# oceanbase/oceanbase

Hardware: AMD Instinct MI355X
Metric: rows/sec, TPC-H lineitem scan->filter->agg (microblock decode + pushdown filter + group-by) (higher is better)
Workload: dtype int64; 1 GPU; tpch_q1_sf100_lineitem_scan_filter_agg; rows_per_gpu=600000000, total_rows=600000000, encoded_bytes_per_gpu=7341603792, n_blocks=453858, block_bytes=16384

## Files before the change

include/obx.h:

```cpp
#ifndef OBX_H_
#define OBX_H_

#include <stdint.h>
#include <stddef.h>

#ifdef __cplusplus
extern "C" {
#endif

enum {
  OBX_SUCCESS = 0,
  OBX_ITER_END = -4008,
  OBX_INVALID_ARGUMENT = -4002,
  OBX_NOT_SUPPORTED = -4007,
  OBX_BUF_NOT_ENOUGH = -4009,
  OBX_NO_GPU = -7001,
  OBX_INTERNAL_ERROR = -4016,
  OBX_PHYSIC_CHECKSUM_ERROR = -4108,
};

enum obx_encoding {
  OBX_ENC_RAW = 0,
  OBX_ENC_DICT = 1,
  OBX_ENC_RLE = 2,
// ... 59 lines not shown
  const obx_col_schema *cols;
  uint64_t total_rows;
} obx_blockset;

#define OBX_MAX_IN_LIST 8
typedef struct obx_filter_leaf {
  uint16_t col;
  uint8_t op;
  uint8_t n_in;
  int64_t lo;
  int64_t hi;
  int64_t in_list[OBX_MAX_IN_LIST];
  int64_t bconst[OBX_BX_MAX_CONST];
  uint16_t bcols[OBX_BX_MAX_COLS];
  uint8_t n_bprog;
  uint8_t n_bcols;
  uint8_t bprog[OBX_BX_MAX_PROG];
  uint8_t bpad[6];
} obx_filter_leaf;

#define OBX_TOK_AND 128
#define OBX_TOK_OR 129
#define OBX_MAX_PROG 15

typedef struct obx_filter_desc {
  uint16_t n_leaves;
  uint8_t n_prog;
  uint8_t prog[OBX_MAX_PROG];
  obx_filter_leaf leaves[8];
} obx_filter_desc;

typedef struct obx_agg_expr {
  uint8_t kind;
  uint16_t col_a;
  uint16_t col_b;
  uint16_t col_c;
} obx_agg_expr;

typedef struct obx_agg_desc {
  uint8_t n_group_cols;
  uint16_t group_cols[2];
  uint8_t n_aggs;
  obx_agg_expr aggs[8];
} obx_agg_desc;

typedef struct obx_agg_cell { uint64_t limb[4]; } obx_agg_cell;

#define OBX_MAX_GROUPS 64
#define OBX_MAX_KEY_BYTES 16
typedef struct obx_group_row {
  uint8_t key[OBX_MAX_KEY_BYTES];
  uint8_t key_len;
  uint64_t row_count;
  obx_agg_cell cells[8];
} obx_group_row;

typedef struct obx_agg_result {
  uint32_t n_groups;
  obx_group_row groups[OBX_MAX_GROUPS];
  uint64_t rows_scanned;
  uint64_t rows_passed;
} obx_agg_result;

typedef struct obx_batch {
  uint64_t *skip_bits;
  int64_t size;
  uint8_t end;
  uint8_t all_rows_active;
} obx_batch;


int64_t obx_encode_block(const obx_col_schema *cols, uint16_t n_cols,
                         const uint8_t *const *col_data,
                         const uint8_t *const *null_bitmaps,
                         uint32_t row_count, const uint8_t *enc_request,
                         uint8_t *out, int64_t out_cap);

uint64_t obx_crc32c(const uint8_t *buf, int64_t len);

int obx_decode_block(const obx_col_schema *cols, uint16_t n_cols,
                     const uint8_t *block, int64_t block_len,
                     const uint16_t *proj_cols, uint16_t n_proj,
                     uint8_t *const *out_cols, uint8_t *const *out_nulls,
                     uint32_t *row_count);

int obx_cpu_filter_block(const obx_col_schema *cols, uint16_t n_cols,
                         const uint8_t *block, int64_t block_len,
                         const obx_filter_desc *filter,
                         uint8_t *result_bits, uint32_t *row_count,
                         uint32_t *popcnt);

int obx_cpu_scan_filter_agg(const obx_blockset *bs,
                            const obx_filter_desc *filter,
                            const obx_agg_desc *agg,
                            int nthreads,
                            obx_agg_result *out);

int64_t obx_gen_lineitem(int config, uint64_t row_count, uint64_t seed,
                         uint32_t target_block_bytes,
                         uint64_t row_id_base,
                         uint8_t **out_data, uint64_t **out_offsets,
                         obx_col_schema *out_cols, uint16_t *out_n_cols);

typedef struct obx_gpu_ctx obx_gpu_ctx;

int obx_gpu_open(int device, obx_gpu_ctx **ctx);
int obx_gpu_close(obx_gpu_ctx *ctx);

int obx_gpu_load_blocks(obx_gpu_ctx *ctx, const obx_blockset *bs);

int obx_gpu_load_cs_blocks(obx_gpu_ctx *ctx, const obx_blockset *bs);

int obx_cs_host_parse(const uint8_t *buf, int64_t len, uint32_t *rows_out,
                      uint32_t *ncols_out);
int obx_gpu_free_blocks(obx_gpu_ctx *ctx, int handle);

int obx_gpu_filter(obx_gpu_ctx *ctx, int handle, const obx_filter_desc *filter,
                   int want_row_ids);
int obx_gpu_fetch_bitmap(obx_gpu_ctx *ctx, int handle, uint8_t *out, int64_t cap);
int obx_gpu_fetch_row_ids(obx_gpu_ctx *ctx, int handle, int32_t *out,
                          int64_t cap, uint64_t *n_out);
int obx_gpu_fetch_blk_counts(obx_gpu_ctx *ctx, int handle, uint32_t *out,
                             int64_t cap);

int obx_gpu_decode(obx_gpu_ctx *ctx, int handle, const uint16_t *proj_cols,
                   uint16_t n_proj);
int obx_gpu_fetch_col(obx_gpu_ctx *ctx, int handle, uint16_t col,
                      uint8_t *out, int64_t cap);

int obx_gpu_scan_project(obx_gpu_ctx *ctx, int handle,
                         const obx_filter_desc *filter,
                         const uint16_t *proj_cols, uint16_t n_proj,
                         int want_row_nos, uint64_t *n_rows);

int obx_gpu_fetch_proj(obx_gpu_ctx *ctx, int handle, uint16_t proj_idx,
                       uint64_t start, uint64_t count,
                       uint8_t *out, int64_t cap,
                       uint8_t *out_nulls, int64_t nulls_cap, uint64_t *n_out);

int obx_gpu_fetch_proj_row_nos(obx_gpu_ctx *ctx, int handle, uint64_t start,
                               uint64_t count, uint64_t *out, int64_t cap,
                               uint64_t *n_out);

double obx_gpu_last_proj_stage_ms(obx_gpu_ctx *ctx, int stage);

int obx_gpu_scan_filter_agg(obx_gpu_ctx *ctx, int handle,
                            const obx_filter_desc *filter,
                            const obx_agg_desc *agg,
                            obx_agg_result *out);

double obx_gpu_last_kernel_ms(obx_gpu_ctx *ctx);
double obx_gpu_last_prep_ms(obx_gpu_ctx *ctx);
int obx_gpu_last_jit(obx_gpu_ctx *ctx);
uint32_t obx_gpu_last_grid(obx_gpu_ctx *ctx);
uint64_t obx_gpu_total_rows(obx_gpu_ctx *ctx, int handle);
uint64_t obx_gpu_total_bytes(obx_gpu_ctx *ctx, int handle);
uint64_t obx_gpu_last_survivors(obx_gpu_ctx *ctx, int handle);

int obx_gpu_agg_fetch(obx_gpu_ctx *ctx, int handle, uint32_t start,
                      uint32_t count, obx_group_row *out, uint32_t *n_out,
                      uint64_t *n_total);
int obx_cpu_agg_fetch(uint32_t start, uint32_t count, obx_group_row *out,
                      uint32_t *n_out, uint64_t *n_total);

int64_t obx_jit_dump_src(const obx_filter_desc *filter,
                         const obx_agg_desc *agg,
                         const obx_col_schema *cols, uint16_t n_cols,
                         const uint8_t *col_flags, const int64_t *col_min,
                         const int64_t *col_max, const uint32_t *col_maxcnt,
                         const uint32_t *col_maxw, uint32_t max_block_rows,
                         int force_v1, char *out, int64_t cap);

#ifdef __cplusplus
}
#endif
#endif
```

oceanbase_amd/csrc/obx_dev.h:

```cpp
#ifndef OBX_DEV_H_
#define OBX_DEV_H_

#if defined(__HIPRTC__) || defined(OBX_HIPRTC)
typedef signed char int8_t;
typedef unsigned char uint8_t;
typedef short int16_t;
typedef unsigned short uint16_t;
typedef int int32_t;
typedef unsigned int uint32_t;
typedef long long int64_t;
typedef unsigned long long uint64_t;
typedef unsigned long size_t;
#define INT64_MAX 0x7fffffffffffffffll
#define INT64_MIN (-INT64_MAX - 1ll)
#define UINT64_MAX 0xffffffffffffffffull
#else
#include <stdint.h>
#endif

#define OBX_DEV_MAX_COLS 8
#define OBX_DEV_MAX_LEAVES 8
#define OBX_DEV_MAX_AGGS 8
#define OBX_GTABLE_SLOTS 256
#define OBX_GTABLE_SHIFT 8
#define OBX_GTABLE_BIG 4096
#define OBX_GTABLE_BIG_SHIFT 12
#define OBX_LTABLE_SLOTS 16

enum {
  OBX_D_RAW = 0,
  OBX_D_DICT = 1,
  OBX_D_RLE = 2,
  OBX_D_CONST = 3,
  OBX_D_INTDIFF = 4,
  OBX_D_SDIFF = 5,
  OBX_D_HEX = 6,
  OBX_D_SPREFIX = 7,
  OBX_D_EQUAL = 8,
  OBX_D_SUBSTR = 9,
};

enum {
  OBX_DF_BITPACK = 1,
  OBX_DF_HAS_EXT = 2,
  OBX_DF_SIGNED = 4,
  OBX_DF_STRING = 8,
};

typedef struct dev_col {
  uint64_t data_bit;
  uint64_t ext_bit;
  uint64_t dict_byte;
  uint64_t aux_byte;
  int64_t base;
  uint32_t count;
  uint32_t runs;
  uint8_t enc;
  uint8_t flags;
  uint8_t width;
  uint8_t entry_len;
  uint8_t rib, rfb;
  uint8_t datum_len;
  uint8_t ext_width;
  uint8_t tss;
  uint8_t pad[7];
} dev_col;

typedef struct dev_block {
  uint32_t row_start_lo;
  uint32_t row_start_hi;
  uint32_t row_count;
  uint32_t block_len;
  uint64_t block_byte;
  dev_col cols[OBX_DEV_MAX_COLS];
} dev_block;

#define OBX_LDS_STAGE_BYTES 17408

#if defined(__HIPCC__) || defined(__HIP_DEVICE_COMPILE__)
__host__ __device__
#endif
static inline uint64_t dev_block_row_start(const dev_block *b) {
  return ((uint64_t)b->row_start_hi << 32) | b->row_start_lo;
}

enum {
  OBX_LEAF_NONE = 0,
  OBX_LEAF_ALL = 1,
  OBX_LEAF_REF_MASK = 2,
  OBX_LEAF_RANGE = 3,
  OBX_LEAF_VALUE = 4,
  OBX_LEAF_NULL = 5,
};

typedef struct dev_leaf {
  int64_t vlo, vhi;
  uint16_t col;
  uint8_t op;
  uint8_t n_in;
  uint8_t char_len;
  uint8_t pad[3];
  int64_t in_list[8];
  int64_t bconst[4];
  uint16_t bcols[4];
  uint8_t n_bprog;
  uint8_t n_bcols;
  uint8_t bprog[24];
  uint8_t bpad[6];
} dev_leaf;

typedef struct blk_leaf {
  uint64_t mask;
  uint64_t lo, hi;
  uint8_t mode;
  uint8_t invert;
  uint8_t pad[6];
} blk_leaf;

typedef struct dev_agg {
  uint8_t kind;
  uint8_t ia, ib, ic;
  int32_t pad;
  int64_t one_b, one_c;
} dev_agg;

#define OBX_DEV_MAX_NEED 12

typedef struct dev_pass_agg {
  uint8_t kind;
  uint8_t agg_idx;
  uint8_t sa, sb, sc;
  uint8_t pad[3];
  int64_t one_b, one_c;
} dev_pass_agg;

typedef struct dev_pass {
  uint8_t n_aggs;
  uint8_t n_cols;
  uint8_t cols[3];
  uint8_t pad[3];
  dev_pass_agg aggs[OBX_DEV_MAX_AGGS];
} dev_pass;

typedef struct dev_plan_hdr {
  uint32_t n_leaves;
  uint32_t n_aggs;
  uint32_t n_group_cols;
  uint32_t n_need;
  uint32_t n_passes;
  uint8_t n_prog;
  uint8_t prog[15];
  uint16_t need_cols[OBX_DEV_MAX_NEED];
  uint8_t group_idx[2];
  uint8_t group_len[2];
  dev_agg aggs[OBX_DEV_MAX_AGGS];
  dev_pass passes[OBX_DEV_MAX_AGGS];
} dev_plan_hdr;

typedef struct gslot {
  unsigned long long key;
  unsigned long long count;
  unsigned long long cells[OBX_DEV_MAX_AGGS][4];
} gslot;

#define OBX_KEY_EMPTY 0xFFFFFFFFFFFFFFFFull

#endif
```

oceanbase_amd/csrc/obx_engine.cpp:

```cpp
#include <cstdlib>
#include <cstring>
#include <algorithm>

#include "obx_host.h"

#define OBX_RESULT_BYTES(slots) (sizeof(gslot) * (slots) + 16 * 8)

extern "C" int obx_gpu_open(int device, obx_gpu_ctx **out) {
  int n = 0;
  hipError_t e = hipGetDeviceCount(&n);
  if (e != hipSuccess || n <= device) return OBX_NO_GPU;
  auto *ctx = new obx_gpu_ctx();
  ctx->device = device;
  HIP_TRY(hipSetDevice(device));
  HIP_TRY(hipStreamCreate(&ctx->stream));
  HIP_TRY(hipEventCreate(&ctx->ev_start));
  HIP_TRY(hipEventCreate(&ctx->ev_stop));
  HIP_TRY(hipEventCreate(&ctx->ev_p0));
  HIP_TRY(hipEventCreate(&ctx->ev_p1));
  HIP_TRY(hipEventCreate(&ctx->ev_mid));
  {
    hipDeviceProp_t prop;
    HIP_TRY(hipGetDeviceProperties(&prop, device));
    if (prop.multiProcessorCount > 0)
      ctx->n_cus = (uint32_t)prop.multiProcessorCount;
  }
  HIP_TRY(hipHostMalloc((void **)&ctx->h_result,
                        OBX_RESULT_BYTES(OBX_GTABLE_BIG), hipHostMallocDefault));
  *out = ctx;
  return OBX_SUCCESS;
}

extern "C" int obx_gpu_close(obx_gpu_ctx *ctx) {
  if (!ctx) return OBX_SUCCESS;
  (void)hipSetDevice(ctx->device);
  ctx->handles.clear();
  (void)hipStreamDestroy(ctx->stream);
  for (hipEvent_t ev : {ctx->ev_start, ctx->ev_stop, ctx->ev_p0, ctx->ev_p1,
                        ctx->ev_mid})
    (void)hipEventDestroy(ev);
  (void)hipHostFree(ctx->h_result);
  delete ctx;
  return OBX_SUCCESS;
}

obx_handle::~obx_handle() {
  void *owned[] = {d_buf, d_blocks, d_bleaves, d_pleaves, d_gtable,
                   d_gtable_big, d_proj_scratch, d_bitmap, d_row_ids,
                   d_blk_counts, d_row_slot, d_minmax, d_sel_nulls,
                   d_sel_row_nos, d_blk_off, d_tile_sums, d_sel_bits};
  for (void *p : owned)
    if (p) (void)hipFree(p);
  for (uint8_t *p : d_decode_out)
    if (p) (void)hipFree(p);
  for (uint8_t *p : d_sel_out)
    if (p) (void)hipFree(p);
}

static obx_handle *lookup(obx_gpu_ctx *ctx, int handle) {
  if (!ctx || handle < 0 || handle >= (int)ctx->handles.size()) return nullptr;
  return ctx->handles[handle].get();
}

__attribute__((target("sse4.2")))
static uint64_t host_crc32c(const uint8_t *buf, int64_t len) {
  uint64_t crc = 0;
  int64_t i = 0;
  for (; i + 8 <= len; i += 8) {
    uint64_t w;
    memcpy(&w, buf + i, 8);
    crc = __builtin_ia32_crc32di(crc, w);
  }
  for (; i < len; i++) crc = __builtin_ia32_crc32qi((uint32_t)crc, buf[i]);
  return crc;
}

#define OBX_JIT_GRID_WAVES 8
static uint32_t jit_grid_for(uint32_t n_blocks, uint32_t n_cus, int wpb) {
  uint64_t g = (uint64_t)(n_cus ? n_cus : 1) * (uint32_t)(wpb > 0 ? wpb : 1) *
               OBX_JIT_GRID_WAVES;
  if (g > n_blocks) g = n_blocks;
  return g ? (uint32_t)g : 1;
}

static void gtable_init(gslot *gt, uint32_t n_slots, uint32_t tail_words,
                        uint32_t min_mask, uint32_t max_mask,
                        hipStream_t stream) {
  const uint32_t words =
      n_slots * (uint32_t)(sizeof(gslot) / 8) + tail_words;
  hipLaunchKernelGGL(k_gtable_init, dim3((words + OBX_WG_HOST - 1) / OBX_WG_HOST),
                     dim3(OBX_WG_HOST), 0, stream, (unsigned long long *)gt,
                     n_slots, tail_words, min_mask, max_mask);
}

static void summarize_col_classes(obx_handle &h) {
  const uint32_t nc = h.n_cols;
  const bool first = h.col_class.size() == nc;
  const uint8_t *cls = h.col_class.data() + h.col_class.size() - nc;
  const uint8_t *cnt = h.col_cnt.data() + h.col_cnt.size() - nc;
  for (uint32_t c = 0; c < nc; c++) {
    const uint8_t k = cls[c];
    if (first) h.col_grp16_every[c] = true;
    if ((k & 0xF) == 5) h.col_span_any[c] = true;
    if ((k & 0xF) != 1 || cnt[c] >= 16) h.col_grp16_every[c] = false;
    if ((k & 0xF) > 3 || (k & 0x10)) h.col_slow_any[c] = true;
    if (cnt[c] > h.col_cnt_max[c]) h.col_cnt_max[c] = cnt[c];
  }
}

void obx_fold_block(obx_handle &h, const dev_block &db) {
  const bool first = h.col_class.empty();
  if ((db.block_byte & 15) ||
      (uint64_t)db.block_len + 24 > OBX_LDS_STAGE_BYTES ||
      db.row_count > 4096 )
    h.lds_ok = false;
  for (uint16_t c = 0; c < h.n_cols; c++) {
    const dev_col &dc = db.cols[c];
    uint8_t cls;
    switch (dc.enc) {
      case OBX_D_RAW: cls = 0; break;
      case OBX_D_DICT: cls = 1; break;
      case OBX_D_INTDIFF: cls = 2; break;
      case OBX_D_CONST: cls = dc.runs == 0 ? 3 : 4; break;
      case OBX_D_EQUAL: case OBX_D_SUBSTR:
        cls = 5; break;
      default: cls = 4; break;
    }
    if (dc.flags & OBX_DF_STRING) cls |= 0x10;
    h.col_class.push_back(cls);
    h.col_cnt.push_back((uint8_t)(dc.count > 254 ? 255 : dc.count));
    if (first) {
      h.col_dict_every[c] = true;
      h.col_dict_any[c] = true;
      h.col_raw8_every[c] = true;
      h.col_rangefam_every[c] = true;
    }
    if ((cls & 0xF) != 1 || (cls & 0x10) || dc.count > 63)
      h.col_dict_every[c] = false;
    if ((cls & 0xF) != 1 || dc.count > 63)
      h.col_dict_any[c] = false;
    if (!(dc.enc == OBX_D_RAW && !(dc.flags & OBX_DF_BITPACK) &&
          !(dc.flags & OBX_DF_STRING) && !(dc.flags & OBX_DF_HAS_EXT) &&
          dc.width == 8 && (dc.data_bit & 63) == 0))
      h.col_raw8_every[c] = false;
    if (!((dc.enc == OBX_D_RAW || dc.enc == OBX_D_INTDIFF) &&
          !(dc.flags & OBX_DF_STRING) && !(dc.flags & OBX_DF_HAS_EXT)))
      h.col_rangefam_every[c] = false;
    if (dc.count > h.col_maxcnt[c]) h.col_maxcnt[c] = dc.count;
    if (dc.flags & OBX_DF_HAS_EXT) h.col_ext_any[c] = true;
    uint32_t w = 255;
    if (dc.enc == OBX_D_RAW || dc.enc == OBX_D_DICT || dc.enc == OBX_D_INTDIFF)
      w = (dc.flags & OBX_DF_BITPACK) ? dc.width : (uint32_t)dc.width * 8;
    if (w > h.col_maxw[c]) h.col_maxw[c] = w;
  }
  summarize_col_classes(h);
  if (db.row_count > h.max_block_rows) h.max_block_rows = db.row_count;
  if (db.block_len > h.max_block_len) h.max_block_len = db.block_len;
  h.n_blocks++;
  h.total_rows += db.row_count;
}

static int parse_block(const obx_col_schema *cols, uint16_t n_cols,
                       const uint8_t *block, uint64_t dev_off,
                       uint64_t block_len, uint64_t row_start,
                       dev_block *out) {
  const obx_micro_header *h = (const obx_micro_header *)block;
  if (h->magic != OBX_MICRO_BLOCK_MAGIC) return OBX_INVALID_ARGUMENT;
  if (h->column_count != n_cols) return OBX_INVALID_ARGUMENT;
  if (h->data_zlength > (int64_t)block_len ||
      h->data_zlength < OBX_MICRO_HEADER_SIZE)
    return OBX_INVALID_ARGUMENT;
  if ((int64_t)host_crc32c(block + OBX_MICRO_HEADER_SIZE,
                           (int64_t)h->data_zlength - OBX_MICRO_HEADER_SIZE) !=
      h->data_checksum)
    return OBX_PHYSIC_CHECKSUM_ERROR;
  memset(out, 0, sizeof(*out));
  out->row_start_lo = (uint32_t)row_start;
  out->row_start_hi = (uint32_t)(row_start >> 32);
  out->row_count = h->row_count;
  out->block_len = (uint32_t)block_len;
  out->block_byte = dev_off;
  const uint64_t meta_base =
      dev_off + h->header_size + (uint64_t)n_cols * sizeof(obx_col_header);
  const obx_col_header *chp =
      (const obx_col_header *)(block + h->header_size);
  const uint8_t *meta_host = block + h->header_size +
                             (uint64_t)n_cols * sizeof(obx_col_header);
  const uint8_t evb = obx_hdr_extend_value_bit(h);

  for (uint16_t c = 0; c < n_cols; c++) {
    const obx_col_header *ch = &chp[c];
    dev_col *dc = &out->cols[c];
    const int sc = obx_store_class(ch->obj_type);
    const int64_t tss = obx_type_store_size(ch->obj_type);
    dc->enc = (uint8_t)ch->type;
    dc->datum_len = cols[c].len;
    dc->tss = (uint8_t)(tss > 0 ? tss : cols[c].len);
    dc->ext_width = evb;
    if (sc == OBX_SC_INT) dc->flags |= OBX_DF_SIGNED;
    if (sc == OBX_SC_STRING) dc->flags |= OBX_DF_STRING;
    const uint64_t col_base = meta_base + ch->offset;
    const uint8_t *col_host = meta_host + ch->offset;
    const int has_ext = (ch->attr & OBX_COL_ATTR_HAS_EXTEND_VALUE) ? 1 : 0;
    const int bp = (ch->attr & OBX_COL_ATTR_BIT_PACKING) ? 1 : 0;

    switch (ch->type) {
      case OBX_COL_RAW: {
        if (bp) dc->flags |= OBX_DF_BITPACK;
        dc->width = (uint8_t)ch->length;
        uint64_t ext_bits = has_ext ? (uint64_t)evb * h->row_count : 0;
        if (has_ext) {
          dc->flags |= OBX_DF_HAS_EXT;
          dc->ext_bit = col_base * 8;
        }
        if (bp) {
          dc->data_bit = col_base * 8 + ext_bits;
        } else {
          dc->data_bit = (col_base + (ext_bits + 7) / 8) * 8;
        }
        break;
      }
      case OBX_COL_DICT: {
        const obx_dict_meta *dm = (const obx_dict_meta *)col_host;
        if (bp) dc->flags |= OBX_DF_BITPACK;
        dc->width = dm->row_ref_size;
        dc->count = dm->count;
        dc->entry_len = (uint8_t)dm->data_size;
        dc->dict_byte = col_base + sizeof(obx_dict_meta);
        dc->data_bit = (col_base + ch->length) * 8;
        break;
      }
      case OBX_COL_RLE: {
        const obx_rle_meta *rm = (const obx_rle_meta *)col_host;
        dc->runs = rm->count;
        dc->rib = rm->attr & 7;
        dc->rfb = (rm->attr >> 3) & 7;
        dc->aux_byte = col_base + sizeof(obx_rle_meta);
        const obx_dict_meta *dm =
            (const obx_dict_meta *)(col_host + rm->offset);
        dc->count = dm->count;
        dc->entry_len = (uint8_t)dm->data_size;
        dc->dict_byte = col_base + rm->offset + sizeof(obx_dict_meta);
        break;
      }
      case OBX_COL_CONST: {
        const obx_const_meta *cm = (const obx_const_meta *)col_host;
        dc->runs = cm->count;
        dc->rib = cm->attr & 7;
        dc->rfb = cm->const_ref;
        if (cm->count == 0) {
          if (cm->const_ref > 0) {
            dc->count = 0;
          } else {
            dc->count = 1;
            int64_t cell = (sc == OBX_SC_INT) ? tss : cols[c].len;
            uint64_t v = 0;
            memcpy(&v, col_host + cm->offset, (size_t)cell);
            dc->base = (sc == OBX_SC_INT)
                           ? (int64_t)obx_sign_extend(v, tss, 1)
                           : (sc == OBX_SC_DECIMAL
                                  ? (int64_t)obx_sign_extend(v, cell, 1)
                                  : (int64_t)v);
          }
        } else {
          dc->aux_byte = col_base + sizeof(obx_const_meta);
          const obx_dict_meta *dm =
              (const obx_dict_meta *)(col_host + cm->offset);
          dc->count = dm->count;
          dc->entry_len = (uint8_t)dm->data_size;
          dc->dict_byte = col_base + cm->offset + sizeof(obx_dict_meta);
        }
        break;
      }
      case OBX_COL_INTEGER_BASE_DIFF: {
        const obx_intdiff_meta *im = (const obx_intdiff_meta *)col_host;
        if (bp) dc->flags |= OBX_DF_BITPACK;
        dc->width = im->length;
        uint64_t b = 0;
        memcpy(&b, col_host + sizeof(obx_intdiff_meta), (size_t)tss);
        dc->base = (int64_t)obx_sign_extend(b, tss, sc == OBX_SC_INT);
        uint64_t data0 = col_base + ch->length;
        uint64_t ext_bits = has_ext ? (uint64_t)evb * h->row_count : 0;
        if (has_ext) {
          dc->flags |= OBX_DF_HAS_EXT;
          dc->ext_bit = data0 * 8;
        }
        if (bp) dc->data_bit = data0 * 8 + ext_bits;
        else dc->data_bit = (data0 + (ext_bits + 7) / 8) * 8;
        break;
      }
      case OBX_COL_STRING_PREFIX: {
        const obx_sprefix_meta *pm = (const obx_sprefix_meta *)col_host;
        dc->count = pm->count;
        dc->entry_len = pm->hex_char_cnt;
        dc->rib = pm->pib;
        dc->dict_byte = col_base + sizeof(obx_sprefix_meta);
        dc->aux_byte = dc->dict_byte + pm->hex_char_cnt;
        {
          const uint8_t *ends = col_host + sizeof(obx_sprefix_meta) +
                                pm->hex_char_cnt;
          uint64_t prev = 0, min_pl = ~0ull;
          for (uint32_t j = 0; j < pm->count; j++) {
            uint64_t e2 = 0;
            memcpy(&e2, ends + (size_t)j * pm->pib, pm->pib);
            if (e2 - prev < min_pl) min_pl = e2 - prev;
            prev = e2;
// ... 252 lines not shown
    for (uint16_t i = 0; i < nl; i++) {
      if (pl[i].op != OBX_OP_GE && pl[i].op != OBX_OP_GT) continue;
      for (uint16_t k = 0; k < nl; k++) {
        if (k == i || pl[k].col != pl[i].col) continue;
        if (pl[k].op != OBX_OP_LE && pl[k].op != OBX_OP_LT) continue;
        int64_t lo = pl[i].vlo, hi = pl[k].vlo;
        if (pl[i].op == OBX_OP_GT) {
          if (lo == INT64_MAX) continue;
          lo++;
        }
        if (pl[k].op == OBX_OP_LT) {
          if (hi == INT64_MIN) continue;
          hi--;
        }
        pl[i].op = OBX_OP_BT;
        pl[i].vlo = lo;
        pl[i].vhi = hi;
        for (uint16_t m = k; m + 1 < nl; m++) pl[m] = pl[m + 1];
        nl--;
        ph.n_leaves = nl;
        if (k < i) i--;
        i--;
        break;
      }
    }
  }

  int slot_of_col[64];
  for (int i = 0; i < 64; i++) slot_of_col[i] = -1;
  auto need = [&](uint16_t c) -> uint8_t {
    if (slot_of_col[c] < 0) {
      if (ph.n_need >= OBX_DEV_MAX_NEED) return 0xFF;
      slot_of_col[c] = ph.n_need;
      ph.need_cols[ph.n_need++] = c;
    }
    return (uint8_t)slot_of_col[c];
  };
  if (agg) {
    if (agg->n_group_cols > 2 || agg->n_aggs > OBX_DEV_MAX_AGGS)
      return OBX_INVALID_ARGUMENT;
    ph.n_group_cols = agg->n_group_cols;
    for (int g = 0; g < agg->n_group_cols; g++) {
      if (agg->group_cols[g] >= h.n_cols) return OBX_INVALID_ARGUMENT;
      ph.group_idx[g] = need(agg->group_cols[g]);
      ph.group_len[g] = h.cols[agg->group_cols[g]].len;
    }
    ph.n_aggs = agg->n_aggs;
    for (int a = 0; a < agg->n_aggs; a++) {
      const obx_agg_expr *e = &agg->aggs[a];
      dev_agg *da = &ph.aggs[a];
      da->kind = e->kind;
      da->ia = da->ib = da->ic = 0xFF;
      if (e->col_a != UINT16_MAX && e->col_a >= h.n_cols)
        return OBX_INVALID_ARGUMENT;
      if (e->col_a != UINT16_MAX) da->ia = need(e->col_a);
      if (e->kind == OBX_AGG_SUM_PROD2 || e->kind == OBX_AGG_SUM_PROD3 ||
          e->kind == OBX_AGG_SUM_MUL) {
        if (e->col_b >= h.n_cols) return OBX_INVALID_ARGUMENT;
        da->ib = need(e->col_b);
        static const int64_t P10[19] = {1ll,10ll,100ll,1000ll,10000ll,
          100000ll,1000000ll,10000000ll,100000000ll,1000000000ll,
          10000000000ll,100000000000ll,1000000000000ll,10000000000000ll,
          100000000000000ll,1000000000000000ll,10000000000000000ll,
          100000000000000000ll,1000000000000000000ll};
        da->one_b = P10[h.cols[e->col_b].scale];
        if (e->kind == OBX_AGG_SUM_PROD3) {
          if (e->col_c >= h.n_cols) return OBX_INVALID_ARGUMENT;
          da->ic = need(e->col_c);
          da->one_c = P10[h.cols[e->col_c].scale];
        }
      }
    }
    for (uint32_t g = 0; g < ph.n_group_cols; g++)
      if (h.col_span_any[ph.need_cols[ph.group_idx[g]]])
        return OBX_NOT_SUPPORTED;
  }
  if (agg) {
    bool used[OBX_DEV_MAX_AGGS] = {};
    ph.n_passes = 0;
    for (int a = 0; a < agg->n_aggs; a++) {
      if (used[a]) continue;
      const dev_agg *da = &ph.aggs[a];
      if (da->kind == OBX_AGG_COUNT && da->ia == 0xFF) { used[a] = true; continue; }
      dev_pass *pp = &ph.passes[ph.n_passes++];
      memset(pp, 0, sizeof(*pp));
      auto col_sel = [&](uint8_t need_idx) -> int {
        if (need_idx == 0xFF) return -1;
        for (int k = 0; k < pp->n_cols; k++)
          if (pp->cols[k] == need_idx) return k;
        if (pp->n_cols >= 3) return -2;
        pp->cols[pp->n_cols] = need_idx;
        return pp->n_cols++;
      };
      auto try_add = [&](int idx) -> bool {
        const dev_agg *d = &ph.aggs[idx];
        uint8_t save_n = pp->n_cols;
        int sa = col_sel(d->ia), sb = col_sel(d->ib), sc = col_sel(d->ic);
        if (sa == -2 || sb == -2 || sc == -2) { pp->n_cols = save_n; return false; }
        dev_pass_agg *pa = &pp->aggs[pp->n_aggs++];
        pa->kind = d->kind;
        pa->agg_idx = (uint8_t)idx;
        pa->sa = (uint8_t)(sa < 0 ? 0xFF : sa);
        pa->sb = (uint8_t)(sb < 0 ? 0xFF : sb);
        pa->sc = (uint8_t)(sc < 0 ? 0xFF : sc);
        pa->one_b = d->one_b;
        pa->one_c = d->one_c;
        return true;
      };
      try_add(a);
      used[a] = true;
      for (int b2 = a + 1; b2 < agg->n_aggs; b2++) {
        if (used[b2]) continue;
        const dev_agg *d2 = &ph.aggs[b2];
        if (d2->kind == OBX_AGG_COUNT && d2->ia == 0xFF) { used[b2] = true; continue; }
        if (try_add(b2)) used[b2] = true;
      }
    }
  }

  return OBX_SUCCESS;
}

static int prep_query(obx_gpu_ctx *ctx, obx_handle &h,
                      const obx_filter_desc *filter, const obx_agg_desc *agg,
                      dev_plan_hdr &ph, dev_leaf *pl_out = nullptr) {
  dev_leaf pl[OBX_DEV_MAX_LEAVES];
  int rc = build_plan(h, filter, agg, ph, pl);
  if (pl_out) memcpy(pl_out, pl, sizeof(pl));
  if (rc != OBX_SUCCESS) return rc;
  uint16_t nl = ph.n_leaves;
  HIP_TRY(hipEventRecord(ctx->ev_p0, ctx->stream));
  HIP_TRY(hipMemcpyAsync(h.d_pleaves, pl, sizeof(pl), hipMemcpyHostToDevice,
                         ctx->stream));
  if (nl > 0) {
    uint64_t needed = (uint64_t)h.n_blocks * nl;
    if (h.bleaves_cap < needed) {
      (void)hipFree(h.d_bleaves);
      h.d_bleaves = nullptr;
      h.bleaves_cap = 0;
      HIP_TRY(hipMalloc(&h.d_bleaves, needed * sizeof(blk_leaf)));
      h.bleaves_cap = needed;
    }
    uint32_t total = (uint32_t)needed;
    uint32_t grid = (total + OBX_WG_HOST - 1) / OBX_WG_HOST;
    hipLaunchKernelGGL(k_lower_leaves, dim3(grid), dim3(OBX_WG_HOST), 0, ctx->stream,
                       h.d_buf, h.d_blocks, h.n_blocks, h.d_pleaves, nl,
                       (uint32_t)h.n_cols, (const int64_t *)h.d_minmax,
                       h.d_bleaves);
  }
  HIP_TRY(hipEventRecord(ctx->ev_p1, ctx->stream));
  return OBX_SUCCESS;
}

#include "obx_jit.inc"

static decltype(&k_filter) generic_filter_kernel(const obx_handle &h,
                                                 const dev_plan_hdr &ph) {
  return h.lds_ok ? (ph.n_prog ? k_filter_prog_lds : k_filter_lds)
                  : (ph.n_prog ? k_filter_prog : k_filter);
}

static int end_timed(obx_gpu_ctx *ctx, bool prep, const void *result = nullptr,
                     size_t result_bytes = 0) {
  HIP_TRY(hipEventRecord(ctx->ev_stop, ctx->stream));
  if (result)
    HIP_TRY(hipMemcpyAsync(ctx->h_result, result, result_bytes,
                           hipMemcpyDeviceToHost, ctx->stream));
  HIP_TRY(hipStreamSynchronize(ctx->stream));
  float ms = 0;
  HIP_TRY(hipEventElapsedTime(&ms, ctx->ev_start, ctx->ev_stop));
  ctx->last_ms = ms;
  if (prep) {
    HIP_TRY(hipEventElapsedTime(&ms, ctx->ev_p0, ctx->ev_p1));
    ctx->last_prep_ms = ms;
  }
  return OBX_SUCCESS;
}

static int run_filter(obx_gpu_ctx *ctx, obx_handle &h,
                      const obx_filter_desc *filter, int want_row_ids) {
  HIP_TRY(hipSetDevice(ctx->device));
  dev_plan_hdr ph;
  dev_leaf plv[OBX_DEV_MAX_LEAVES];
  int rc = prep_query(ctx, h, filter, nullptr, ph, plv);
  if (rc != OBX_SUCCESS) return rc;
  ctx->last_jit = 0;
  uint64_t bm_words = (h.total_rows + 63) / 64 + 1;
  if (!h.d_bitmap) HIP_TRY(hipMalloc(&h.d_bitmap, bm_words * 8));
  HIP_TRY(hipMemsetAsync(h.d_bitmap, 0, bm_words * 8, ctx->stream));
  const bool no_bitmap = getenv("OBX_NO_BITMAP") != nullptr;
  if (want_row_ids) {
    if (!h.d_row_ids)
      HIP_TRY(hipMalloc(&h.d_row_ids, h.total_rows * sizeof(int32_t)));
    if (!h.d_blk_counts)
      HIP_TRY(hipMalloc(&h.d_blk_counts, h.n_blocks * sizeof(uint32_t)));
    HIP_TRY(hipMemsetAsync(h.d_blk_counts, 0,
                           h.n_blocks * sizeof(uint32_t), ctx->stream));
  }
  HIP_TRY(hipMemsetAsync(h.d_counters, 0, 16 * 8, ctx->stream));
  jit_entry *fje = jit_prepare_filter(h, ph, plv, want_row_ids);
  ctx->last_jit = fje ? 2 : 0;
  HIP_TRY(hipEventRecord(ctx->ev_start, ctx->stream));
  if (fje) {
    uint32_t fgrid = h.n_blocks / 8;
    if (fgrid < 512) fgrid = h.n_blocks < 512 ? (h.n_blocks ? h.n_blocks : 1)
                                              : 512;
    if (fgrid > 2048) fgrid = 2048;
    if (const char *fg = getenv("OBX_JIT_FGRID")) {
      int g = atoi(fg);
      if (g > 0 && g <= 65535) fgrid = (uint32_t)g;
    }
    void *rid = want_row_ids ? (void *)h.d_row_ids : nullptr;
    void *bcn = want_row_ids ? (void *)h.d_blk_counts : nullptr;
    void *args[9] = {&h.d_buf, &h.d_blocks, &h.n_blocks, &h.d_pleaves,
                     &h.d_bleaves, &h.d_bitmap, &rid, &bcn, &h.d_counters};
    if (hipModuleLaunchKernel(fje->fn, fgrid, 1, 1,
                              OBX_WG_HOST, 1, 1, 0, ctx->stream, args,
                              nullptr) != hipSuccess)
      return OBX_INTERNAL_ERROR;
  } else {
    hipLaunchKernelGGL(generic_filter_kernel(h, ph),
                       dim3(grid_for(h.n_blocks)), dim3(OBX_WG_HOST), 0,
                       ctx->stream, h.d_buf, h.d_blocks, h.n_blocks,
                       h.d_pleaves, h.d_bleaves, ph,
                       (h.lds_ok && no_bitmap) ? nullptr : h.d_bitmap,
                       want_row_ids ? h.d_row_ids : nullptr,
                       want_row_ids ? h.d_blk_counts : nullptr, h.d_counters);
  }
  rc = end_timed(ctx, true);
  if (rc != OBX_SUCCESS) return rc;
  unsigned long long cnt[16];
  HIP_TRY(hipMemcpy(cnt, h.d_counters, 16 * 8, hipMemcpyDeviceToHost));
  h.last_survivors = cnt[0];
  for (int i2 = 8; i2 < 16; i2++) h.last_survivors += cnt[i2];
  return OBX_SUCCESS;
}

extern "C" int obx_gpu_filter(obx_gpu_ctx *ctx, int handle,
                              const obx_filter_desc *filter,
                              int want_row_ids) {
  obx_handle *hp = lookup(ctx, handle);
  if (!hp) return OBX_INVALID_ARGUMENT;
  return run_filter(ctx, *hp, filter, want_row_ids);
}

extern "C" int obx_gpu_fetch_bitmap(obx_gpu_ctx *ctx, int handle, uint8_t *out,
                                    int64_t cap) {
  obx_handle *hp = lookup(ctx, handle);
  if (!hp) return OBX_INVALID_ARGUMENT;
  obx_handle &h = *hp;
  if (!h.d_bitmap) return OBX_INVALID_ARGUMENT;
  int64_t bytes = (int64_t)((h.total_rows + 7) / 8);
  if (cap < bytes) return OBX_BUF_NOT_ENOUGH;
  HIP_TRY(hipMemcpy(out, h.d_bitmap, bytes, hipMemcpyDeviceToHost));
  return OBX_SUCCESS;
}

extern "C" int obx_gpu_fetch_row_ids(obx_gpu_ctx *ctx, int handle,
                                     int32_t *out, int64_t cap,
                                     uint64_t *n_out) {
  obx_handle *hp = lookup(ctx, handle);
  if (!hp) return OBX_INVALID_ARGUMENT;
  obx_handle &h = *hp;
  if (!h.d_row_ids) return OBX_INVALID_ARGUMENT;
  if (n_out) *n_out = h.last_survivors;
  if (out) {
    if (cap < (int64_t)h.total_rows) return OBX_BUF_NOT_ENOUGH;
    HIP_TRY(hipMemcpy(out, h.d_row_ids, h.total_rows * sizeof(int32_t),
                      hipMemcpyDeviceToHost));
  }
  return OBX_SUCCESS;
}

extern "C" int obx_gpu_fetch_blk_counts(obx_gpu_ctx *ctx, int handle,
                                        uint32_t *out, int64_t cap) {
  obx_handle *hp = lookup(ctx, handle);
  if (!hp) return OBX_INVALID_ARGUMENT;
  obx_handle &h = *hp;
  if (!h.d_blk_counts) return OBX_INVALID_ARGUMENT;
  if (cap < (int64_t)h.n_blocks) return OBX_BUF_NOT_ENOUGH;
  HIP_TRY(hipMemcpy(out, h.d_blk_counts, h.n_blocks * 4,
                    hipMemcpyDeviceToHost));
  return OBX_SUCCESS;
}

extern "C" int obx_gpu_decode(obx_gpu_ctx *ctx, int handle,
                              const uint16_t *proj_cols, uint16_t n_proj) {
  obx_handle *hp = lookup(ctx, handle);
  if (!hp) return OBX_INVALID_ARGUMENT;
  obx_handle &h = *hp;
  HIP_TRY(hipSetDevice(ctx->device));
  HIP_TRY(hipEventRecord(ctx->ev_start, ctx->stream));
  if (h.lds_ok && n_proj > 1 && n_proj <= OBX_DEV_MAX_COLS) {
    uint16_t pc[OBX_DEV_MAX_COLS];
    uint8_t ln[OBX_DEV_MAX_COLS];
    uint8_t *po[OBX_DEV_MAX_COLS];
    for (uint16_t i = 0; i < n_proj; i++) {
      uint16_t c = proj_cols[i];
      if (c >= h.n_cols) return OBX_INVALID_ARGUMENT;
      if (!h.d_decode_out[c])
        HIP_TRY(hipMalloc(&h.d_decode_out[c], h.total_rows * h.cols[c].len));
      pc[i] = c;
      ln[i] = (uint8_t)h.cols[c].len;
      po[i] = h.d_decode_out[c];
    }
    if (!h.d_proj_scratch)
      HIP_TRY(hipMalloc(&h.d_proj_scratch,
                        OBX_DEV_MAX_COLS * (8 + 2 + 1) + 16));
    uint8_t *base = (uint8_t *)h.d_proj_scratch;
    uint8_t *outp = base;
    uint8_t *pcp = base + OBX_DEV_MAX_COLS * 8;
    uint8_t *lnp = pcp + OBX_DEV_MAX_COLS * 2;
    HIP_TRY(hipMemcpy(outp, po, sizeof(void *) * n_proj,
                      hipMemcpyHostToDevice));
    HIP_TRY(hipMemcpy(pcp, pc, sizeof(uint16_t) * n_proj,
                      hipMemcpyHostToDevice));
    HIP_TRY(hipMemcpy(lnp, ln, n_proj, hipMemcpyHostToDevice));
    hipLaunchKernelGGL(k_decode_multi, dim3(grid_for(h.n_blocks)),
                       dim3(OBX_WG_HOST), 0, ctx->stream, h.d_buf,
                       h.d_blocks, h.n_blocks, (const uint16_t *)pcp,
                       lnp, (uint32_t)n_proj, (uint8_t *const *)outp,
                       (uint8_t *const *)nullptr);
  } else {
    for (uint16_t i = 0; i < n_proj; i++) {
      uint16_t c = proj_cols[i];
      if (c >= h.n_cols) return OBX_INVALID_ARGUMENT;
      if (!h.d_decode_out[c])
// ... 49 lines not shown
  uint64_t total = h.total_rows;
  ctx->last_proj_ms[0] = ctx->last_proj_ms[1] = ctx->last_proj_ms[2] = 0.0;
  if (filtered) {
    int rc = run_filter(ctx, h, filter, 1);
    if (rc != OBX_SUCCESS) return rc;
    ctx->last_proj_ms[0] = ctx->last_ms;
    total = h.last_survivors;
  } else {
    ctx->last_jit = 0;
  }

  if (total > 0) {
    proj_args pa;
    memset(&pa, 0, sizeof(pa));
    pa.n_proj = n_proj;
    for (uint16_t i = 0; i < n_proj; i++) {
      const uint16_t c = proj_cols[i];
      int rc = grow(h.d_sel_out[i], h.sel_out_cap[i], total * h.cols[c].len, 1);
      if (rc != OBX_SUCCESS) return rc;
      pa.out[i] = h.d_sel_out[i];
      pa.col[i] = c;
      pa.len[i] = h.cols[c].len;
    }
    int rc = grow(h.d_sel_nulls, h.sel_nulls_cap, total, 1);
    if (rc != OBX_SUCCESS) return rc;
    if (want_row_nos) {
      rc = grow(h.d_sel_row_nos, h.sel_row_nos_cap, total, sizeof(uint64_t));
      if (rc != OBX_SUCCESS) return rc;
    }
    const uint32_t n_tiles = (h.n_blocks + OBX_PROJ_TILE - 1) / OBX_PROJ_TILE;
    if (filtered && !h.d_blk_off) {
      HIP_TRY(hipMalloc(&h.d_blk_off, ((uint64_t)h.n_blocks + 1) * 8));
      HIP_TRY(hipMalloc(&h.d_tile_sums, (uint64_t)n_tiles * 8));
    }

    HIP_TRY(hipEventRecord(ctx->ev_start, ctx->stream));
    if (filtered) {
      hipLaunchKernelGGL(k_project_tile_sums, dim3(n_tiles), dim3(OBX_WG_HOST),
                         0, ctx->stream, h.d_blk_counts, h.n_blocks,
                         h.d_tile_sums);
      hipLaunchKernelGGL(k_project_offsets, dim3(n_tiles), dim3(OBX_WG_HOST),
                         0, ctx->stream, h.d_blk_counts, h.n_blocks,
                         h.d_tile_sums, h.d_blk_off);
    }
    HIP_TRY(hipEventRecord(ctx->ev_mid, ctx->stream));
    hipLaunchKernelGGL(h.lds_ok ? k_project_sel_lds : k_project_sel,
                       dim3(grid_for(h.n_blocks)), dim3(OBX_WG_HOST), 0,
                       ctx->stream, h.d_buf, h.d_blocks, h.n_blocks,
                       filtered ? h.d_row_ids : (const int32_t *)nullptr,
                       filtered ? h.d_blk_counts : (const uint32_t *)nullptr,
                       filtered ? h.d_blk_off : (const uint64_t *)nullptr, pa,
                       h.d_sel_nulls,
                       want_row_nos ? h.d_sel_row_nos : (uint64_t *)nullptr,
                       total);
    rc = end_timed(ctx, false);
    if (rc != OBX_SUCCESS) return rc;
    float ms = 0;
    HIP_TRY(hipEventElapsedTime(&ms, ctx->ev_start, ctx->ev_mid));
    ctx->last_proj_ms[1] = ms;
    HIP_TRY(hipEventElapsedTime(&ms, ctx->ev_mid, ctx->ev_stop));
    ctx->last_proj_ms[2] = ms;
  }
  ctx->last_ms = ctx->last_proj_ms[0] + ctx->last_proj_ms[1] +
                 ctx->last_proj_ms[2];

  memcpy(h.sel_cols, proj_cols, sizeof(uint16_t) * n_proj);
  h.sel_has_row_nos = want_row_nos != 0;
  h.sel_rows = total;
  h.sel_n_proj = n_proj;
  if (n_rows) *n_rows = total;
  return OBX_SUCCESS;
}

static uint64_t sel_window(const obx_handle &h, uint64_t start,
                           uint64_t count) {
  if (start >= h.sel_rows) return 0;
  return count < h.sel_rows - start ? count : h.sel_rows - start;
}

extern "C" int obx_gpu_fetch_proj(obx_gpu_ctx *ctx, int handle,
                                  uint16_t proj_idx, uint64_t start,
                                  uint64_t count, uint8_t *out, int64_t cap,
                                  uint8_t *out_nulls, int64_t nulls_cap,
                                  uint64_t *n_out) {
  obx_handle *hp = lookup(ctx, handle);
  if (!hp) return OBX_INVALID_ARGUMENT;
  obx_handle &h = *hp;
  if (proj_idx >= h.sel_n_proj) return OBX_INVALID_ARGUMENT;
  const uint64_t n = sel_window(h, start, count);
  if (n_out) *n_out = n;
  if (n == 0) return OBX_SUCCESS;
  const uint64_t len = h.cols[h.sel_cols[proj_idx]].len;
  const uint64_t null_bytes = (n + 7) / 8;
  if (out && (cap < 0 || (uint64_t)cap < n * len)) return OBX_BUF_NOT_ENOUGH;
  if (out_nulls && (nulls_cap < 0 || (uint64_t)nulls_cap < null_bytes))
    return OBX_BUF_NOT_ENOUGH;
  HIP_TRY(hipSetDevice(ctx->device));
  if (out)
    HIP_TRY(hipMemcpyAsync(out, h.d_sel_out[proj_idx] + start * len, n * len,
                           hipMemcpyDeviceToHost, ctx->stream));
  if (out_nulls) {
    int rc = grow(h.d_sel_bits, h.sel_bits_cap, null_bytes, 1);
    if (rc != OBX_SUCCESS) return rc;
    uint64_t g = (null_bytes + OBX_WG_HOST - 1) / OBX_WG_HOST;
    if (g > 4096) g = 4096;
    hipLaunchKernelGGL(k_project_pack_nulls, dim3((uint32_t)g),
                       dim3(OBX_WG_HOST), 0, ctx->stream, h.d_sel_nulls,
                       start, n, (uint32_t)proj_idx, h.d_sel_bits);
    HIP_TRY(hipMemcpyAsync(out_nulls, h.d_sel_bits, null_bytes,
                           hipMemcpyDeviceToHost, ctx->stream));
  }
  HIP_TRY(hipStreamSynchronize(ctx->stream));
  return OBX_SUCCESS;
}

extern "C" int obx_gpu_fetch_proj_row_nos(obx_gpu_ctx *ctx, int handle,
                                          uint64_t start, uint64_t count,
                                          uint64_t *out, int64_t cap,
                                          uint64_t *n_out) {
  obx_handle *hp = lookup(ctx, handle);
  if (!hp) return OBX_INVALID_ARGUMENT;
  obx_handle &h = *hp;
  if (!h.sel_n_proj || !h.sel_has_row_nos) return OBX_INVALID_ARGUMENT;
  const uint64_t n = sel_window(h, start, count);
  if (n_out) *n_out = n;
  if (n == 0 || !out) return OBX_SUCCESS;
  if (cap < 0 || (uint64_t)cap < n) return OBX_BUF_NOT_ENOUGH;
  HIP_TRY(hipSetDevice(ctx->device));
  HIP_TRY(hipMemcpyAsync(out, h.d_sel_row_nos + start, n * sizeof(uint64_t),
                         hipMemcpyDeviceToHost, ctx->stream));
  HIP_TRY(hipStreamSynchronize(ctx->stream));
  return OBX_SUCCESS;
}

extern "C" double obx_gpu_last_proj_stage_ms(obx_gpu_ctx *ctx, int stage) {
  return ctx && stage >= 0 && stage < 3 ? ctx->last_proj_ms[stage] : -1.0;
}

extern "C" int obx_gpu_scan_filter_agg(obx_gpu_ctx *ctx, int handle,
                                       const obx_filter_desc *filter,
                                       const obx_agg_desc *agg,
                                       obx_agg_result *out) {
  obx_handle *hp = lookup(ctx, handle);
  if (!hp || !out) return OBX_INVALID_ARGUMENT;
  obx_handle &h = *hp;
  HIP_TRY(hipSetDevice(ctx->device));
  h.last_rows.clear();
  dev_plan_hdr ph;
  dev_leaf plv[OBX_DEV_MAX_LEAVES];
  int rc = prep_query(ctx, h, filter, agg, ph, plv);
  if (rc != OBX_SUCCESS) return rc;
  ctx->last_jit = 0;
  ctx->last_grid = 0;

  uint32_t min_mask = 0, max_mask = 0;
  for (uint32_t a = 0; a < ph.n_aggs; a++) {
    if (ph.aggs[a].kind == OBX_AGG_MIN) min_mask |= 1u << a;
    else if (ph.aggs[a].kind == OBX_AGG_MAX) max_mask |= 1u << a;
  }
  gtable_init(h.d_gtable, OBX_GTABLE_SLOTS, 16, min_mask, max_mask,
              ctx->stream);

  const bool use_pipeline = getenv("OBX_PIPELINE_AGG") != nullptr;
  if (use_pipeline) {
    uint64_t bm_words = (h.total_rows + 63) / 64 + 1;
    if (!h.d_bitmap) HIP_TRY(hipMalloc(&h.d_bitmap, bm_words * 8));
    HIP_TRY(hipMemsetAsync(h.d_bitmap, 0, bm_words * 8, ctx->stream));
    if (!h.d_row_slot) HIP_TRY(hipMalloc(&h.d_row_slot, h.total_rows + 1));

    HIP_TRY(hipEventRecord(ctx->ev_start, ctx->stream));
    hipLaunchKernelGGL(generic_filter_kernel(h, ph),
                       dim3(grid_for(h.n_blocks)), dim3(OBX_WG_HOST), 0,
                       ctx->stream, h.d_buf, h.d_blocks, h.n_blocks,
                       h.d_pleaves, h.d_bleaves, ph, h.d_bitmap,
                       (int32_t *)nullptr, (uint32_t *)nullptr, h.d_counters);
    hipLaunchKernelGGL(k_group_pass, dim3(grid_for(h.n_blocks)),
                       dim3(OBX_WG_HOST), 0, ctx->stream, h.d_buf, h.d_blocks,
                       h.n_blocks, ph, h.d_bitmap, h.d_row_slot, h.d_gtable,
                       h.d_counters);
    for (uint32_t a = 0; a < ph.n_aggs;) {
      const dev_agg &ag = ph.aggs[a];
      if (ag.kind == OBX_AGG_COUNT && ag.ia == 0xFF) { a++; continue; }
      bool fuse = (ag.kind == OBX_AGG_SUM_PROD2 && a + 1 < ph.n_aggs &&
                   ph.aggs[a + 1].kind == OBX_AGG_SUM_PROD3 &&
                   ph.aggs[a + 1].ia == ag.ia && ph.aggs[a + 1].ib == ag.ib);
      hipLaunchKernelGGL(k_agg_pass, dim3(grid_for(h.n_blocks)),
                         dim3(OBX_WG_HOST), 0, ctx->stream, h.d_buf,
                         h.d_blocks, h.n_blocks, ph, a, h.d_bitmap,
                         h.d_row_slot, h.d_gtable);
      a += fuse ? 2 : 1;
    }
  } else {
    jit_entry *je = jit_prepare(h, ph, plv);
    ctx->last_jit = je ? g_jit_kind : 0;
    HIP_TRY(hipEventRecord(ctx->ev_start, ctx->stream));
    if (je) {
      if (jit_launch(je, h, ctx->stream, &ctx->last_grid) != 0)
        return OBX_INTERNAL_ERROR;
    } else {
      auto kfn = h.lds_ok
                     ? (ph.n_prog ? k_scan_filter_agg_prog_lds
                                  : k_scan_filter_agg_lds)
                     : (ph.n_prog ? k_scan_filter_agg_prog : k_scan_filter_agg);
      hipLaunchKernelGGL(kfn, dim3(grid_for(h.n_blocks)), dim3(OBX_WG_HOST), 0,
                         ctx->stream, h.d_buf, h.d_blocks, h.n_blocks,
                         h.d_pleaves, h.d_bleaves, ph, h.d_gtable,
                         h.d_counters);
    }
  }
  rc = end_timed(ctx, true, h.d_gtable, OBX_RESULT_BYTES(OBX_GTABLE_SLOTS));
  if (rc != OBX_SUCCESS) return rc;

  const gslot *gt = (const gslot *)ctx->h_result;
  size_t n_gt = OBX_GTABLE_SLOTS;
  unsigned long long cnt[16];
  memcpy(cnt, gt + OBX_GTABLE_SLOTS, sizeof(cnt));
  if (cnt[1] != 0) {
    if (ph.n_prog != 0) return OBX_BUF_NOT_ENOUGH;
    if (!h.d_gtable_big)
      HIP_TRY(hipMalloc(&h.d_gtable_big, OBX_RESULT_BYTES(OBX_GTABLE_BIG)));
    unsigned long long *big_counters =
        (unsigned long long *)(h.d_gtable_big + OBX_GTABLE_BIG);
    gtable_init(h.d_gtable_big, OBX_GTABLE_BIG, 16, min_mask, max_mask,
                ctx->stream);
    hipLaunchKernelGGL(k_scan_agg_direct, dim3(grid_for(h.n_blocks)),
                       dim3(OBX_WG_HOST), 0, ctx->stream, h.d_buf,
                       h.d_blocks, h.n_blocks, h.d_pleaves, h.d_bleaves,
                       ph, h.d_gtable_big, big_counters);
    HIP_TRY(hipMemcpyAsync(ctx->h_result, h.d_gtable_big,
                           OBX_RESULT_BYTES(OBX_GTABLE_BIG),
                           hipMemcpyDeviceToHost, ctx->stream));
    HIP_TRY(hipStreamSynchronize(ctx->stream));
    n_gt = OBX_GTABLE_BIG;
    memcpy(cnt, gt + OBX_GTABLE_BIG, sizeof(cnt));
    if (cnt[2] != 0) return OBX_BUF_NOT_ENOUGH;
  }
  for (int i2 = 8; i2 < 16; i2++) cnt[0] += cnt[i2];

  memset(out, 0, sizeof(*out));
  out->rows_scanned = h.total_rows;
  out->rows_passed = cnt[0];
  uint8_t key_len = 0;
  if (agg)
    for (int g = 0; g < agg->n_group_cols; g++)
      key_len += h.cols[agg->group_cols[g]].len;
  std::vector<const gslot *> live;
  for (size_t i = 0; i < n_gt; i++)
    if (gt[i].key != OBX_KEY_EMPTY) live.push_back(&gt[i]);
  std::sort(live.begin(), live.end(), [](const gslot *a, const gslot *b) {
    uint8_t ka[8], kb[8];
    memcpy(ka, &a->key, 8);
    memcpy(kb, &b->key, 8);
    return memcmp(ka, kb, 8) < 0;
  });
  h.last_rows.assign(live.size(), obx_group_row());
  for (size_t i = 0; i < live.size(); i++) {
    obx_group_row *g = &h.last_rows[i];
    memcpy(g->key, &live[i]->key, 8);
    g->key_len = key_len;
    g->row_count = live[i]->count;
    uint32_t na = agg ? agg->n_aggs : 0;
    for (uint32_t a = 0; a < na; a++) {
      uint8_t kind = agg->aggs[a].kind;
      if (kind == OBX_AGG_COUNT && agg->aggs[a].col_a == UINT16_MAX) {
        g->cells[a].limb[0] = live[i]->count;
        g->cells[a].limb[1] = g->cells[a].limb[2] = g->cells[a].limb[3] = 0;
      } else if (kind == OBX_AGG_MIN || kind == OBX_AGG_MAX) {
        int64_t v = live[i]->cells[a][1] ? (int64_t)live[i]->cells[a][0] : 0;
        g->cells[a].limb[0] = (uint64_t)v;
        uint64_t s = v < 0 ? ~0ull : 0ull;
        g->cells[a].limb[1] = g->cells[a].limb[2] = g->cells[a].limb[3] = s;
      } else {
        for (int l = 0; l < 4; l++)
          g->cells[a].limb[l] = live[i]->cells[a][l];
      }
    }
  }
  if (h.last_rows.size() > OBX_MAX_GROUPS) {
    out->n_groups = (uint32_t)h.last_rows.size();
    return OBX_BUF_NOT_ENOUGH;
  }
  out->n_groups = (uint32_t)h.last_rows.size();
  for (size_t i = 0; i < h.last_rows.size(); i++)
    out->groups[i] = h.last_rows[i];
  return OBX_SUCCESS;
}

extern "C" uint64_t obx_crc32c(const uint8_t *buf, int64_t len) {
  return host_crc32c(buf, len);
}

extern "C" int64_t obx_jit_dump_src_ex(
    const obx_filter_desc *filter, const obx_agg_desc *agg,
    const obx_col_schema *cols, uint16_t n_cols, const uint8_t *col_flags,
    const int64_t *col_min, const int64_t *col_max,
    const uint32_t *col_maxcnt, const uint32_t *col_maxw,
    uint32_t max_block_rows, int force_v1, uint32_t n_blocks, uint32_t n_cus,
    uint32_t *grid_out, char *out, int64_t cap) {
  if (!cols || n_cols > OBX_DEV_MAX_COLS) return OBX_INVALID_ARGUMENT;
  if (grid_out) *grid_out = 0;
  obx_handle h;
  h.n_cols = n_cols;
  h.n_blocks = n_blocks ? n_blocks : 1;
  if (n_cus) h.n_cus = n_cus;
  h.max_block_rows = max_block_rows ? max_block_rows : 4096;
  h.max_block_len = OBX_LDS_STAGE_BYTES - 32;
  memcpy(h.cols, cols, sizeof(obx_col_schema) * n_cols);
  for (uint16_t c = 0; c < n_cols; c++) {
    h.col_dict_every[c] = (col_flags[c] & 1) != 0;
    h.col_ext_any[c] = (col_flags[c] & 2) != 0;
    h.col_known[c] = (col_flags[c] & 4) != 0;
    h.col_raw8_every[c] = (col_flags[c] & 8) != 0;
    h.col_rangefam_every[c] = (col_flags[c] & 16) != 0;
    h.col_dict_any[c] = h.col_dict_every[c] ||
        (obx_store_class(cols[c].obj_type) == OBX_SC_STRING &&
         (col_flags[c] & 1));
    h.col_dict_stable[c] = (col_flags[c] & 32) != 0 && h.col_dict_any[c];
    h.col_min[c] = col_min[c];
    h.col_max[c] = col_max[c];
    h.col_maxcnt[c] = col_maxcnt[c];
    h.col_maxw[c] = col_maxw ? col_maxw[c] : 255;
    uint8_t cls = h.col_dict_every[c] ? 1 : 0;
    if (obx_store_class(cols[c].obj_type) == OBX_SC_STRING) cls |= 0x10;
    h.col_class.push_back(cls);
    h.col_cnt.push_back(
        (uint8_t)(h.col_maxcnt[c] > 254 ? 255 : h.col_maxcnt[c]));
  }
  summarize_col_classes(h);
  dev_plan_hdr ph;
  dev_leaf pl[OBX_DEV_MAX_LEAVES];
  int rc = build_plan(h, filter, agg, ph, pl);
  if (rc != OBX_SUCCESS) return rc;
  if (!agg) {
    jit_fstrategy fst;
    if (!jit_build_fstrategy(h, ph, pl, fst)) return 0;
    if (getenv("OBX_DUMP_RID") && fst.fstage) {
      fst.frid = 1;
      fst.fnch = (uint16_t)((h.max_block_rows + 63) / 64);
    }
    std::string fsrc = jit_gen_source_filter(ph, fst);
    if (out && cap > (int64_t)fsrc.size()) {
      memcpy(out, fsrc.data(), fsrc.size());
      out[fsrc.size()] = 0;
    }
    return (int64_t)fsrc.size();
  }
  jit_shape js;
  if (!jit_plan_shape(ph, js)) return 0;
  if (!jit_blocks_ok(h, ph, js)) return 0;
  jit_strategy st;
  if (!force_v1) jit_build_strategy(h, ph, js, pl, st);
  if (!st.ok && js.has_mm) return 0;
  if (st.ok && grid_out)
    *grid_out = jit_grid_for(h.n_blocks, h.n_cus, st.wpb);
  std::string src = st.ok ? jit_gen_source_v2(ph, js, st)
                          : jit_gen_source(ph, js);
  if (out && cap > (int64_t)src.size()) {
    memcpy(out, src.data(), src.size());
    out[src.size()] = 0;
  }
  return (int64_t)src.size();
}

extern "C" int64_t obx_jit_dump_src(
    const obx_filter_desc *filter, const obx_agg_desc *agg,
    const obx_col_schema *cols, uint16_t n_cols, const uint8_t *col_flags,
    const int64_t *col_min, const int64_t *col_max,
    const uint32_t *col_maxcnt, const uint32_t *col_maxw,
    uint32_t max_block_rows, int force_v1,
    char *out, int64_t cap) {
  return obx_jit_dump_src_ex(filter, agg, cols, n_cols, col_flags, col_min,
                             col_max, col_maxcnt, col_maxw, max_block_rows,
                             force_v1, 1, 0, nullptr, out, cap);
}

extern "C" int obx_jit_probe_blocks(
    const obx_filter_desc *filter, const obx_agg_desc *agg,
    const obx_col_schema *cols, uint16_t n_cols, const uint8_t *col_class,
    const uint8_t *col_cnt, uint32_t n_blocks) {
  if (!cols || !col_class || !col_cnt || n_cols > OBX_DEV_MAX_COLS)
    return OBX_INVALID_ARGUMENT;
  obx_handle h;
  h.n_cols = n_cols;
  h.n_blocks = n_blocks;
  memcpy(h.cols, cols, sizeof(obx_col_schema) * n_cols);
  for (size_t b = 0; b < n_blocks; b++) {
    h.col_class.insert(h.col_class.end(), col_class + b * n_cols,
                       col_class + (b + 1) * n_cols);
    h.col_cnt.insert(h.col_cnt.end(), col_cnt + b * n_cols,
                     col_cnt + (b + 1) * n_cols);
    summarize_col_classes(h);
  }
  dev_plan_hdr ph;
  dev_leaf pl[OBX_DEV_MAX_LEAVES];
  int rc = build_plan(h, filter, agg, ph, pl);
  if (rc != OBX_SUCCESS) return rc;
  jit_shape js;
  return jit_plan_shape(ph, js) && jit_blocks_ok(h, ph, js) ? 1 : 0;
}

extern "C" int obx_probe_load_facts(const obx_blockset *bs, int is_cs,
                                    uint64_t *handle_out, uint32_t *col_out) {
  if (!bs || !handle_out || !col_out) return OBX_INVALID_ARGUMENT;
  obx_handle h;
  std::vector<dev_block> blocks;
  int rc = is_cs ? obx_cs_host_load(bs, h, blocks, nullptr)
                 : obx_pax_host_load(bs, h, blocks);
  if (rc != OBX_SUCCESS) return rc;
  const uint64_t hf[7] = {h.n_blocks, h.n_cols, h.total_rows, h.total_bytes,
                          h.lds_ok, h.max_block_rows, h.max_block_len};
  memcpy(handle_out, hf, sizeof(hf));
  for (uint16_t c = 0; c < h.n_cols; c++) {
    const bool f[9] = {h.col_dict_every[c], h.col_dict_any[c],
                       h.col_dict_stable[c], h.col_grp16_every[c],
                       h.col_raw8_every[c], h.col_rangefam_every[c],
                       h.col_ext_any[c], h.col_slow_any[c], h.col_span_any[c]};
    uint32_t *o = col_out + 4 * c;
    o[0] = 0;
    for (int i = 0; i < 9; i++) o[0] |= (uint32_t)f[i] << i;
    o[1] = h.col_maxcnt[c];
    o[2] = h.col_maxw[c];
    o[3] = h.col_cnt_max[c];
  }
  return OBX_SUCCESS;
}

extern "C" double obx_gpu_last_kernel_ms(obx_gpu_ctx *ctx) {
  return ctx ? ctx->last_ms : -1.0;
}

extern "C" double obx_gpu_last_prep_ms(obx_gpu_ctx *ctx) {
  return ctx ? ctx->last_prep_ms : -1.0;
}

extern "C" int obx_gpu_last_jit(obx_gpu_ctx *ctx) {
  return ctx ? ctx->last_jit : 0;
}

extern "C" uint32_t obx_gpu_last_grid(obx_gpu_ctx *ctx) {
  return ctx ? ctx->last_grid : 0;
}

extern "C" uint64_t obx_gpu_total_rows(obx_gpu_ctx *ctx, int handle) {
  const obx_handle *h = lookup(ctx, handle);
  return h ? h->total_rows : 0;
}
extern "C" uint64_t obx_gpu_total_bytes(obx_gpu_ctx *ctx, int handle) {
  const obx_handle *h = lookup(ctx, handle);
  return h ? h->total_bytes : 0;
}
extern "C" uint64_t obx_gpu_last_survivors(obx_gpu_ctx *ctx, int handle) {
  const obx_handle *h = lookup(ctx, handle);
  return h ? h->last_survivors : 0;
}

extern "C" int obx_gpu_agg_fetch(obx_gpu_ctx *ctx, int handle,
                                 uint32_t start, uint32_t count,
                                 obx_group_row *out, uint32_t *n_out,
                                 uint64_t *n_total) {
  obx_handle *hp = lookup(ctx, handle);
  if (!hp || !out) return OBX_INVALID_ARGUMENT;
  obx_handle &h = *hp;
  uint64_t total = h.last_rows.size();
  if (n_total) *n_total = total;
  uint32_t n = 0;
  for (; n < count && start + n < total; n++) out[n] = h.last_rows[start + n];
  if (n_out) *n_out = n;
  return OBX_SUCCESS;
}
```

oceanbase_amd/csrc/obx_host.h:

```cpp
#ifndef OBX_HOST_H_
#define OBX_HOST_H_

#include <hip/hip_runtime.h>

#include <cstdio>
#include <map>
#include <memory>
#include <vector>

#include "obx_dev.h"
#include "obx_project.h"

#define OBX_WG_HOST 256

#include "../../include/obx.h"
#include "../../oracle/obx_format.h"

extern "C" __global__ void k_decode_lds(
    const uint8_t *, const dev_block *, uint32_t, uint32_t, uint32_t,
    uint8_t *, uint8_t *);
extern "C" __global__ void k_decode_multi(
    const uint8_t *, const dev_block *, uint32_t, const uint16_t *,
    const uint8_t *, uint32_t, uint8_t *const *, uint8_t *const *);
extern "C" __global__ void k_scan_agg_direct(
    const uint8_t *, const dev_block *, uint32_t, const dev_leaf *,
    const blk_leaf *, const dev_plan_hdr, gslot *, unsigned long long *);
extern "C" __global__ void k_scan_filter_agg(
    const uint8_t *, const dev_block *, uint32_t, const dev_leaf *,
    const blk_leaf *, const dev_plan_hdr, gslot *, unsigned long long *);
extern "C" __global__ void k_scan_filter_agg_lds(
    const uint8_t *, const dev_block *, uint32_t, const dev_leaf *,
    const blk_leaf *, const dev_plan_hdr, gslot *, unsigned long long *);
extern "C" __global__ void k_filter(
    const uint8_t *, const dev_block *, uint32_t, const dev_leaf *,
    const blk_leaf *, const dev_plan_hdr, uint64_t *, int32_t *, uint32_t *,
    unsigned long long *);
extern "C" __global__ void k_filter_lds(
    const uint8_t *, const dev_block *, uint32_t, const dev_leaf *,
    const blk_leaf *, const dev_plan_hdr, uint64_t *, int32_t *, uint32_t *,
    unsigned long long *);
extern "C" __global__ void k_scan_filter_agg_prog(
    const uint8_t *, const dev_block *, uint32_t, const dev_leaf *,
    const blk_leaf *, const dev_plan_hdr, gslot *, unsigned long long *);
extern "C" __global__ void k_scan_filter_agg_prog_lds(
    const uint8_t *, const dev_block *, uint32_t, const dev_leaf *,
    const blk_leaf *, const dev_plan_hdr, gslot *, unsigned long long *);
extern "C" __global__ void k_filter_prog(
    const uint8_t *, const dev_block *, uint32_t, const dev_leaf *,
    const blk_leaf *, const dev_plan_hdr, uint64_t *, int32_t *, uint32_t *,
    unsigned long long *);
extern "C" __global__ void k_filter_prog_lds(
    const uint8_t *, const dev_block *, uint32_t, const dev_leaf *,
    const blk_leaf *, const dev_plan_hdr, uint64_t *, int32_t *, uint32_t *,
    unsigned long long *);
extern "C" __global__ void k_decode(
    const uint8_t *, const dev_block *, uint32_t, uint32_t, uint32_t,
    uint8_t *, uint8_t *);
extern "C" __global__ void k_group_pass(
    const uint8_t *, const dev_block *, uint32_t, const dev_plan_hdr,
    const uint64_t *, uint8_t *, gslot *, unsigned long long *);
extern "C" __global__ void k_agg_pass(
    const uint8_t *, const dev_block *, uint32_t, const dev_plan_hdr,
    uint32_t, const uint64_t *, const uint8_t *, gslot *);
extern "C" __global__ void k_lower_leaves(
    const uint8_t *, const dev_block *, uint32_t, const dev_leaf *, uint32_t,
    uint32_t, const int64_t *, blk_leaf *);
extern "C" __global__ void k_col_minmax(
    const uint8_t *, const dev_block *, uint32_t, uint32_t, int64_t *);
extern "C" __global__ void k_gtable_init(
    unsigned long long *, uint32_t, uint32_t, uint32_t, uint32_t);

extern "C" __global__ void k_project_tile_sums(const uint32_t *, uint32_t,
                                               uint64_t *);
extern "C" __global__ void k_project_offsets(const uint32_t *, uint32_t,
                                             const uint64_t *, uint64_t *);
extern "C" __global__ void k_project_sel(
    const uint8_t *, const dev_block *, uint32_t, const int32_t *,
    const uint32_t *, const uint64_t *, const proj_args, uint8_t *,
    uint64_t *, uint64_t);
extern "C" __global__ void k_project_sel_lds(
    const uint8_t *, const dev_block *, uint32_t, const int32_t *,
    const uint32_t *, const uint64_t *, const proj_args, uint8_t *,
    uint64_t *, uint64_t);
extern "C" __global__ void k_project_pack_nulls(const uint8_t *, uint64_t,
                                                uint64_t, uint32_t, uint8_t *);

#define HIP_TRY(x)                                        \
  do {                                                    \
    hipError_t _e = (x);                                  \
    if (_e != hipSuccess) {                               \
      fprintf(stderr, "obx: HIP error %s at %s:%d\n",     \
              hipGetErrorString(_e), __FILE__, __LINE__); \
      return OBX_INTERNAL_ERROR;                          \
    }                                                     \
  } while (0)

template <class T>
struct dev_tmp {
  T *p = nullptr;
  dev_tmp() = default;
  dev_tmp(const dev_tmp &) = delete;
  dev_tmp &operator=(const dev_tmp &) = delete;
  ~dev_tmp() { if (p) (void)hipFree(p); }
};

struct obx_handle {
  obx_handle() = default;
  obx_handle(const obx_handle &) = delete;
  obx_handle &operator=(const obx_handle &) = delete;
  ~obx_handle();

  uint8_t *d_buf = nullptr;
  dev_block *d_blocks = nullptr;
  uint32_t n_blocks = 0;
  uint16_t n_cols = 0;
  uint64_t total_rows = 0;
  uint64_t total_bytes = 0;
  obx_col_schema cols[OBX_DEV_MAX_COLS];
  blk_leaf *d_bleaves = nullptr;
  uint32_t bleaves_cap = 0;
  dev_leaf *d_pleaves = nullptr;
  gslot *d_gtable = nullptr;
  unsigned long long *d_counters = nullptr;
  uint64_t *d_bitmap = nullptr;
  int32_t *d_row_ids = nullptr;
  uint32_t *d_blk_counts = nullptr;
  uint8_t *d_row_slot = nullptr;
  uint8_t *d_decode_out[OBX_DEV_MAX_COLS] = {};
  uint64_t last_survivors = 0;
  gslot *d_gtable_big = nullptr;
  void *d_proj_scratch = nullptr;
  uint8_t *d_sel_out[OBX_DEV_MAX_COLS] = {};
  uint64_t sel_out_cap[OBX_DEV_MAX_COLS] = {};
  uint8_t *d_sel_nulls = nullptr;
  uint64_t *d_sel_row_nos = nullptr;
  uint64_t sel_nulls_cap = 0, sel_row_nos_cap = 0;
  uint64_t *d_blk_off = nullptr;
  uint64_t *d_tile_sums = nullptr;
  uint8_t *d_sel_bits = nullptr;
  uint64_t sel_bits_cap = 0;
  uint16_t sel_cols[OBX_DEV_MAX_COLS] = {};
  uint16_t sel_n_proj = 0;
  bool sel_has_row_nos = false;
  uint64_t sel_rows = 0;
  std::vector<obx_group_row> last_rows;
  uint32_t n_cus = 256;

  bool lds_ok = true;
  uint32_t max_block_rows = 0;
  uint32_t max_block_len = 0;
  std::vector<uint8_t> col_class, col_cnt;
  bool col_span_any[OBX_DEV_MAX_COLS] = {};
  bool col_grp16_every[OBX_DEV_MAX_COLS] = {};
  bool col_slow_any[OBX_DEV_MAX_COLS] = {};
  uint32_t col_cnt_max[OBX_DEV_MAX_COLS] = {};
  mutable std::map<uint32_t, uint32_t> pair_cells_max;
  bool col_dict_every[OBX_DEV_MAX_COLS] = {};
  bool col_dict_any[OBX_DEV_MAX_COLS] = {};
  bool col_dict_stable[OBX_DEV_MAX_COLS] = {};
  bool col_ext_any[OBX_DEV_MAX_COLS] = {};
  bool col_raw8_every[OBX_DEV_MAX_COLS] = {};
  bool col_rangefam_every[OBX_DEV_MAX_COLS] = {};
  uint32_t col_maxcnt[OBX_DEV_MAX_COLS] = {};
  uint32_t col_maxw[OBX_DEV_MAX_COLS] = {};

  int64_t *d_minmax = nullptr;
  int64_t col_min[OBX_DEV_MAX_COLS] = {};
  int64_t col_max[OBX_DEV_MAX_COLS] = {};
  bool col_known[OBX_DEV_MAX_COLS] = {};
};

struct obx_gpu_ctx {
  int device = 0;
  hipStream_t stream = nullptr;
  hipEvent_t ev_start = nullptr, ev_stop = nullptr;
  hipEvent_t ev_p0 = nullptr, ev_p1 = nullptr;
  hipEvent_t ev_mid = nullptr;
  double last_ms = 0.0;
  double last_prep_ms = 0.0;
  int last_jit = 0;
  double last_proj_ms[3] = {0.0, 0.0, 0.0};
  uint32_t last_grid = 0;
  uint32_t n_cus = 256;
  uint8_t *h_result = nullptr;
  std::vector<std::unique_ptr<obx_handle>> handles;
};

static inline uint32_t grid_for(uint32_t n_blocks) {
  uint32_t g = n_blocks < 4096u ? n_blocks : 4096u;
  return g ? g : 1;
}


void obx_fold_block(obx_handle &h, const dev_block &db);

int obx_finish_load(obx_gpu_ctx *ctx, std::unique_ptr<obx_handle> h,
                    const std::vector<dev_block> &blocks);

int obx_pax_host_load(const obx_blockset *bs, obx_handle &h,
                      std::vector<dev_block> &blocks);
struct obx_cs_plan;
int obx_cs_host_load(const obx_blockset *bs, obx_handle &h,
                     std::vector<dev_block> &blocks,
                     obx_cs_plan *plan );

#endif
```

oceanbase_amd/csrc/obx_jit.inc:

```

#include <hip/hiprtc.h>

#include <map>
#include <string>

struct jit_entry {
  hipModule_t mod = nullptr;
  hipFunction_t fn = nullptr;
  int wpb = 0;
};

struct jit_shape {
  int n_vc = 0;
  uint8_t vcol[4] = {0xFF, 0xFF, 0xFF, 0xFF};
  int n_wa = 0;
  uint8_t agg_wa[OBX_DEV_MAX_AGGS];
  uint8_t agg_f2 = 0;
  bool has_mm = false;
};

#include "obx_jit_scan_v1.inc"
#include "obx_jit_scan.inc"
#include "obx_jit_filter.inc"

static const char *OBX_JIT_SRC_DEV_H =
#include "obx_embed_dev_h.inc"
    ;
static const char *OBX_JIT_SRC_COMMON_H =
#include "obx_embed_common_h.inc"
    ;
static const char *OBX_JIT_SRC_JIT_DEV_H =
#include "obx_embed_jit_dev_h.inc"
    ;

static std::map<std::string, jit_entry> g_jit_cache;
static int g_jit_kind = 0;

static bool jit_plan_shape(const dev_plan_hdr &ph, jit_shape &js) {
  if (ph.n_prog || ph.n_aggs == 0) return false;
  auto vc_add = [&](uint8_t need_idx) -> bool {
    if (need_idx == 0xFF) return true;
    uint8_t col = ph.need_cols[need_idx];
    for (int j = 0; j < js.n_vc; j++)
      if (js.vcol[j] == col) return true;
    if (js.n_vc >= 4) return false;
    js.vcol[js.n_vc++] = col;
    return true;
  };
  for (uint32_t a = 0; a < ph.n_aggs; a++) {
    const dev_agg &g = ph.aggs[a];
    js.agg_wa[a] = 0xFF;
    if (g.kind == OBX_AGG_COUNT && g.ia == 0xFF) continue;
    if (g.kind == OBX_AGG_MIN || g.kind == OBX_AGG_MAX) {
      js.has_mm = true;
      if (!vc_add(g.ia)) return false;
      continue;
    }
    if (g.kind != OBX_AGG_COUNT && g.kind != OBX_AGG_SUM &&
        g.kind != OBX_AGG_SUM_PROD2 && g.kind != OBX_AGG_SUM_PROD3 &&
        g.kind != OBX_AGG_SUM_MUL)
      return false;
    bool f2 = (g.kind == OBX_AGG_SUM_PROD2 && a + 1 < ph.n_aggs &&
               ph.aggs[a + 1].kind == OBX_AGG_SUM_PROD3 &&
               ph.aggs[a + 1].ia == g.ia && ph.aggs[a + 1].ib == g.ib);
    js.agg_wa[a] = (uint8_t)js.n_wa;
    if (!vc_add(g.ia) || !vc_add(g.ib) ||
        !vc_add(f2 ? ph.aggs[a + 1].ic : g.ic))
      return false;
    if (f2) {
      js.agg_f2 |= (uint8_t)(1u << a);
      js.agg_wa[a + 1] = (uint8_t)(js.n_wa + 1);
      a++;
    }
    js.n_wa += f2 ? 2 : 1;
  }
  return js.n_wa <= 8;
}

static uint32_t jit_pair_cells_max(const obx_handle &h, uint8_t c0,
                                   uint8_t c1) {
  const uint32_t key = ((uint32_t)c0 << 16) | c1;
  auto it = h.pair_cells_max.find(key);
  if (it != h.pair_cells_max.end()) return it->second;
  const uint32_t nc = h.n_cols;
  uint32_t mx = 0;
  for (uint32_t b = 0; b < h.n_blocks; b++) {
    const uint8_t *cnt = &h.col_cnt[(size_t)b * nc];
    uint32_t cells = ((uint32_t)cnt[c0] + 1) * ((uint32_t)cnt[c1] + 1);
    if (cells > mx) mx = cells;
  }
  h.pair_cells_max[key] = mx;
  return mx;
}

static bool jit_blocks_ok(const obx_handle &h, const dev_plan_hdr &ph,
                          const jit_shape &js) {
  if (!h.lds_ok || h.col_class.empty()) return false;
  uint8_t gcol[2] = {0xFF, 0xFF};
  uint32_t cells = 1;
  for (uint32_t g = 0; g < ph.n_group_cols; g++) {
    gcol[g] = ph.need_cols[ph.group_idx[g]];
    if (!h.col_grp16_every[gcol[g]]) return false;
    cells *= h.col_cnt_max[gcol[g]] + 1;
  }
  if (cells > 16 && (ph.n_group_cols < 2 ||
                     jit_pair_cells_max(h, gcol[0], gcol[1]) > 16))
    return false;
  for (int j = 0; j < js.n_vc; j++)
    if (h.col_slow_any[js.vcol[j]]) return false;
  return true;
}

template <class GenSrc>
static jit_entry *jit_get(const std::string &key, GenSrc &&gen_src,
                          const char *kernel, const char *dump_name,
                          int wpb) {
  auto it = g_jit_cache.find(key);
  if (it != g_jit_cache.end())
    return it->second.fn ? &it->second : nullptr;
  jit_entry &ent = g_jit_cache[key];
  ent.wpb = wpb;
  const std::string src = gen_src();
  if (const char *dump_dir = getenv("OBX_JIT_DUMP")) {
    FILE *f = fopen((std::string(dump_dir) + "/" + dump_name).c_str(), "w");
    if (!f) f = fopen((std::string("/tmp/") + dump_name).c_str(), "w");
    if (f) { fwrite(src.data(), 1, src.size(), f); fclose(f); }
  }
  hiprtcProgram prog;
  const char *hdrs[3] = {OBX_JIT_SRC_COMMON_H, OBX_JIT_SRC_DEV_H,
                         OBX_JIT_SRC_JIT_DEV_H};
  const char *hdr_names[3] = {"obx_dev_common.h", "obx_dev.h",
                              "obx_jit_dev.h"};
  if (hiprtcCreateProgram(&prog, src.c_str(), dump_name, 3, hdrs,
                          hdr_names) != HIPRTC_SUCCESS)
    return nullptr;
  const char *opts[] = {"--offload-arch=gfx950", "-O3", "-std=c++17",
                        "-DOBX_HIPRTC=1"};
  if (hiprtcCompileProgram(prog, 4, opts) != HIPRTC_SUCCESS) {
    size_t lsz = 0;
    hiprtcGetProgramLogSize(prog, &lsz);
    if (lsz > 1) {
      std::string log(lsz, '\0');
      hiprtcGetProgramLog(prog, &log[0]);
      fprintf(stderr, "obx: JIT compile failed (%s):\n%s\n", kernel,
              log.c_str());
    }
    hiprtcDestroyProgram(&prog);
    return nullptr;
  }
  size_t csz = 0;
  hiprtcGetCodeSize(prog, &csz);
  std::string code(csz, '\0');
  hiprtcGetCode(prog, &code[0]);
  hiprtcDestroyProgram(&prog);
  if (hipModuleLoadData(&ent.mod, code.data()) != hipSuccess ||
      hipModuleGetFunction(&ent.fn, ent.mod, kernel) != hipSuccess) {
    fprintf(stderr, "obx: JIT module load failed (%s)\n", kernel);
    ent.fn = nullptr;
    return nullptr;
  }
  return &ent;
}

static jit_entry *jit_prepare(const obx_handle &h, const dev_plan_hdr &ph,
                              const dev_leaf *pl) {
  const char *e = getenv("OBX_JIT");
  if (e && e[0] == '0') return nullptr;
  jit_shape js;
  if (!jit_plan_shape(ph, js)) return nullptr;
  if (!jit_blocks_ok(h, ph, js)) return nullptr;
  jit_strategy st;
  jit_build_strategy(h, ph, js, pl, st);
  if (!st.ok && js.has_mm) return nullptr;
  g_jit_kind = st.ok ? 2 : 1;
  return jit_get(
      jit_plan_sig(ph) + (st.ok ? jit_strategy_sig(st) : "V1|"),
      [&] {
        return st.ok ? jit_gen_source_v2(ph, js, st) : jit_gen_source(ph, js);
      },
      "k_jit_scan", "obx_jit_src.hip", st.ok ? st.wpb : 0);
}

static jit_entry *jit_prepare_filter(const obx_handle &h,
                                     const dev_plan_hdr &ph,
                                     const dev_leaf *pl, int want_row_ids) {
  const char *e = getenv("OBX_JIT");
  if (e && e[0] == '0') return nullptr;
  jit_fstrategy st;
  if (!jit_build_fstrategy(h, ph, pl, st)) return nullptr;
  if (want_row_ids) {
    uint32_t nch = ((h.max_block_rows ? h.max_block_rows : 4096) + 63) / 64;
    if (!st.fstage || nch > 256) return nullptr;
    st.frid = 1;
    st.fnch = (uint16_t)nch;
  }
  return jit_get(
      jit_fstrategy_sig(ph, st), [&] { return jit_gen_source_filter(ph, st); },
      "k_jit_filter", "obx_jit_filter_src.hip", 0);
}

static int jit_launch(jit_entry *je, obx_handle &h, hipStream_t stream,
                      uint32_t *grid_out) {
  const uint32_t grid = je->wpb ? jit_grid_for(h.n_blocks, h.n_cus, je->wpb)
                                : grid_for(h.n_blocks);
  *grid_out = grid;
  void *args[7] = {&h.d_buf,     &h.d_blocks, &h.n_blocks, &h.d_pleaves,
                   &h.d_bleaves, &h.d_gtable, &h.d_counters};
  return hipModuleLaunchKernel(je->fn, grid, 1, 1, OBX_WG_HOST, 1, 1, 0,
                               stream, args, nullptr) == hipSuccess
             ? 0
             : -1;
}
```

oceanbase_amd/csrc/obx_jit_dev.h:

```cpp
#ifndef OBX_JIT_DEV_H
#define OBX_JIT_DEV_H

#define PW(dc)                                              \
  (((dc).flags & OBX_DF_BITPACK) ? (uint32_t)(dc).width     \
                                 : (uint32_t)(dc).width * 8u)

__device__ __forceinline__ void stage2(
    const uint8_t *__restrict__ buf, const dev_block &blk,
    uint8_t *dst) {
  const uint32_t n16 = (blk.block_len + 15) >> 4;
  const uint8_t *src = buf + blk.block_byte;
  for (uint32_t i = threadIdx.x; i < n16; i += WG) {
    __builtin_amdgcn_global_load_lds(
        (const __attribute__((address_space(1))) uint32_t
             *)(src + (size_t)i * 16),
        (__attribute__((address_space(3))) uint32_t
             *)(dst + (size_t)i * 16),
        16, 0, 0);
  }
}

__device__ __forceinline__ uint64_t jit_bread(
    const uint8_t *__restrict__ b, uint32_t bitpos, uint32_t k) {
  const uint64_t *w = (const uint64_t *)b;
  uint32_t widx = bitpos >> 6, sh = bitpos & 63;
  uint64_t v = w[widx] >> sh;
  if (sh + k > 64) v |= w[widx + 1] << (64 - sh);
  if (k < 64) v &= (((uint64_t)1 << k) - 1);
  return v;
}

__device__ __forceinline__ uint32_t jit_bread32(
    const uint8_t *__restrict__ b, uint32_t bitpos) {
  const uint32_t *w = (const uint32_t *)b;
  const uint32_t widx = bitpos >> 5;
  return __builtin_amdgcn_alignbit(w[widx + 1], w[widx], bitpos & 31);
}

__device__ __forceinline__ int jit_gslot(gslot *gt, uint64_t key) {
  uint32_t idx = (uint32_t)((key * 0x9E3779B97F4A7C15ull) >>
                            (64 - OBX_GTABLE_SHIFT)) &
                 (OBX_GTABLE_SLOTS - 1);
  for (int probe = 0; probe < OBX_GTABLE_SLOTS; probe++) {
    unsigned long long ck = atomicCAS(&gt[idx].key, OBX_KEY_EMPTY,
                                      (unsigned long long)key);
    if (ck == OBX_KEY_EMPTY || ck == key) return (int)idx;
    idx = (idx + 1) & (OBX_GTABLE_SLOTS - 1);
  }
  return -1;
}

__device__ __forceinline__ uint8_t f3and(uint8_t a, uint8_t b) {
  return (a == 0 || b == 0) ? 0 : ((a == 1 && b == 1) ? 1 : 2);
}
__device__ __forceinline__ uint8_t f3or(uint8_t a, uint8_t b) {
  return (a == 1 || b == 1) ? 1 : ((a == 0 && b == 0) ? 0 : 2);
}

#endif
```

oceanbase_amd/csrc/obx_jit_scan.inc:

```

enum { JV_CTX = 0, JV_REF = 1 };
enum {
  JA_COUNT_STAR = 0,
  JA_I64 = 1,
  JA_HIST = 2,
  JA_HCOUNT = 3,
  JA_I64_COUNT = 4,
  JA_MM = 5,
  JA_HISTMM = 6,
};

struct jit_vtab {
  uint8_t vc;
  uint8_t kind;
  int64_t one;
  uint32_t dim;
};

struct jit_strategy {
  bool ok = false;
  uint8_t vmode[4] = {};
  uint8_t vext[4] = {};
  uint8_t vraw8[4] = {};
  uint32_t vdim[4] = {};
  uint8_t astrat[OBX_DEV_MAX_AGGS] = {};
  int8_t wa64[OBX_DEV_MAX_AGGS];
  int8_t amm[OBX_DEV_MAX_AGGS];
  int n_mm = 0;
  int8_t ahist[OBX_DEV_MAX_AGGS];
  int8_t atab_b[OBX_DEV_MAX_AGGS];
  int8_t atab_c[OBX_DEV_MAX_AGGS];
  int8_t aval_a[OBX_DEV_MAX_AGGS];
  int8_t atab_a[OBX_DEV_MAX_AGGS];
  int n_w64 = 0;
  int n_hist = 0;
  uint8_t hist_vc[4] = {};
  int8_t hist_tab[4] = {};
  uint32_t hist_off[4] = {};
  uint32_t hist_total = 0;
  int n_tab = 0;
  jit_vtab tabs[6];
  uint8_t leaf_inline = 0;
  uint8_t leaf_kind[8] = {};
  uint16_t leaf_cols[8] = {};
  uint8_t r = 1;
  uint8_t stripes = 4;
  uint32_t stage_bytes = OBX_LDS_STAGE_BYTES + 32;
  uint8_t leaf_multi[8] = {};
  uint8_t g_multi[2] = {};
  uint8_t v_multi[4] = {};
  uint8_t leaf_m32[8] = {};
  uint8_t g_m32[2] = {};
  uint8_t v_m32[4] = {};
  int8_t cnt_hist = -1;
  uint32_t jcells = 16;
  uint8_t jws_on = 0;
  int8_t jws_ja = -1;
  int8_t jws_a0 = -1, jws_a1 = -1;
  uint32_t jws_d0 = 1, jws_d1 = 1;
  uint32_t jws_cells = 16;
  uint8_t jws_member[OBX_DEV_MAX_AGGS] = {};
  int8_t jws_f0[OBX_DEV_MAX_AGGS];
  int8_t jws_f1[OBX_DEV_MAX_AGGS];
  int8_t ctab_agg = -1;
  uint32_t ctab_db = 0, ctab_dc = 0;
  uint32_t lds_bytes = 0;
  int wpb = 7;
};

static bool jit_col_maxabs(const obx_handle &h, uint16_t col, uint64_t *out) {
  if (!h.col_known[col]) return false;
  if (h.col_min[col] > h.col_max[col]) { *out = 0; return true; }
  uint64_t a = h.col_min[col] == INT64_MIN
                   ? (uint64_t)INT64_MAX + 1
                   : (uint64_t)(h.col_min[col] < 0 ? -h.col_min[col]
                                                   : h.col_min[col]);
  uint64_t b2 = (uint64_t)(h.col_max[col] < 0 ? -h.col_max[col]
                                              : h.col_max[col]);
  *out = a > b2 ? a : b2;
  return true;
}

static uint64_t jit_sat_mul(uint64_t a, uint64_t b2) {
  if (a == 0 || b2 == 0) return 0;
  unsigned __int128 p = (unsigned __int128)a * b2;
  const uint64_t SAT = 1ull << 63;
  return p > SAT ? SAT : (uint64_t)p;
}

static int jit_tab_get(jit_strategy &st, uint8_t vc, uint8_t kind,
                       int64_t one, uint32_t dim) {
  for (int t = 0; t < st.n_tab; t++)
    if (st.tabs[t].vc == vc && st.tabs[t].kind == kind &&
        st.tabs[t].one == one)
      return t;
  if (st.n_tab >= 6) return -1;
  st.tabs[st.n_tab] = {vc, kind, one, dim};
  return st.n_tab++;
}

static int jit_hist_get(jit_strategy &st, uint8_t vc, uint32_t dim) {
  for (int t = 0; t < st.n_hist; t++)
    if (st.hist_vc[t] == vc) return t;
  if (st.n_hist >= 4) return -1;
  st.hist_vc[st.n_hist] = vc;
  st.hist_off[st.n_hist] = st.hist_total;
  st.hist_tab[st.n_hist] = -1;
  st.hist_total += st.jcells * dim;
  return st.n_hist++;
}

static bool jit_build_strategy(const obx_handle &h, const dev_plan_hdr &ph,
                               const jit_shape &js, const dev_leaf *pl,
                               jit_strategy &st) {
  const char *e = getenv("OBX_JIT_V2");
  if (e && e[0] == '0') return false;
  if (pl && ph.n_leaves >= 1 && ph.n_leaves <= 4) {
    st.leaf_inline = 1;
    for (uint32_t i = 0; i < ph.n_leaves; i++) {
      uint16_t col = pl[i].col;
      bool mask_ok = pl[i].op != 10 || pl[i].n_bcols == 1;
      if (h.col_dict_any[col] && mask_ok) st.leaf_kind[i] = 2;
      else if (pl[i].op <= 6 && h.col_rangefam_every[col])
        st.leaf_kind[i] = 1;
      else { st.leaf_inline = 0; break; }
      st.leaf_cols[i] = col;
    }
    if (!st.leaf_inline)
      for (uint32_t i = 0; i < 8; i++) st.leaf_kind[i] = 0;
  }
  uint64_t max_term = 0;
  const uint64_t BOUND = 1ull << 62;

  {
    uint32_t cells = 1;
    for (uint32_t g2 = 0; g2 < ph.n_group_cols; g2++)
      cells *= h.col_maxcnt[ph.need_cols[ph.group_idx[g2]]] + 1;
    if (cells < 1) cells = 1;
    if (cells > 16) cells = 16;
    st.jcells = cells;
  }

  for (int j = 0; j < js.n_vc; j++) {
    uint16_t col = js.vcol[j];
    if (h.col_dict_stable[col] && h.col_dict_every[col]) {
      st.vmode[j] = JV_REF;
      st.vdim[j] = h.col_maxcnt[col] + 1;
    } else {
      st.vmode[j] = JV_CTX;
      st.vext[j] = h.col_ext_any[col] ? 1 : 0;
      st.vraw8[j] = h.col_raw8_every[col] ? 1 : 0;
    }
  }
  for (uint32_t g2 = 0; g2 < ph.n_group_cols; g2++)
    if (!h.col_dict_stable[ph.need_cols[ph.group_idx[g2]]]) return false;
  auto slot_of = [&](uint8_t need_idx) -> int {
    if (need_idx == 0xFF) return -1;
    uint16_t col = ph.need_cols[need_idx];
    for (int j = 0; j < js.n_vc; j++)
      if (js.vcol[j] == col) return j;
    return -1;
  };
  auto maxabs_of = [&](uint8_t need_idx, uint64_t *out) -> bool {
    if (need_idx == 0xFF) return false;
    return jit_col_maxabs(h, ph.need_cols[need_idx], out);
  };

  for (uint32_t a = 0; a < ph.n_aggs; a++) {
    const dev_agg &g = ph.aggs[a];
    st.wa64[a] = st.ahist[a] = st.atab_b[a] = st.atab_c[a] = -1;
    st.aval_a[a] = st.atab_a[a] = -1;
    st.amm[a] = -1;
    int ja = slot_of(g.ia), jb = slot_of(g.ib), jc = slot_of(g.ic);
    uint64_t ma = 0, mb = 0, mc = 0;
    switch (g.kind) {
      case OBX_AGG_COUNT:
        if (g.ia == 0xFF) { st.astrat[a] = JA_COUNT_STAR; break; }
        if (ja >= 0 && st.vmode[ja] == JV_REF) {
          int hid = jit_hist_get(st, (uint8_t)ja, st.vdim[ja]);
          if (hid < 0) return false;
          st.astrat[a] = JA_HCOUNT;
          st.ahist[a] = (int8_t)hid;
        } else if (ja >= 0 && !st.vext[ja]) {
          st.astrat[a] = JA_COUNT_STAR;
        } else if (ja >= 0) {
          st.astrat[a] = JA_I64_COUNT;
          st.wa64[a] = (int8_t)st.n_w64++;
          st.aval_a[a] = (int8_t)ja;
        } else {
          return false;
        }
        break;
      case OBX_AGG_SUM:
        if (ja < 0) return false;
        if (st.vmode[ja] == JV_REF) {
          int hid = jit_hist_get(st, (uint8_t)ja, st.vdim[ja]);
          if (hid < 0) return false;
          st.astrat[a] = JA_HIST;
          st.ahist[a] = (int8_t)hid;
        } else {
          if (!maxabs_of(g.ia, &ma)) return false;
          if (ma > max_term) max_term = ma;
          st.astrat[a] = JA_I64;
          st.wa64[a] = (int8_t)st.n_w64++;
          st.aval_a[a] = (int8_t)ja;
        }
        break;
      case OBX_AGG_SUM_PROD2:
      case OBX_AGG_SUM_PROD3:
      case OBX_AGG_SUM_MUL: {
        if (ja < 0 || jb < 0) return false;
        if (!maxabs_of(g.ia, &ma) || !maxabs_of(g.ib, &mb)) return false;
        uint64_t oneb = (uint64_t)(g.one_b < 0 ? -g.one_b : g.one_b);
        uint64_t onec = (uint64_t)(g.one_c < 0 ? -g.one_c : g.one_c);
        uint64_t term;
        if (g.kind == OBX_AGG_SUM_MUL) {
          term = jit_sat_mul(ma, mb);
        } else {
          term = jit_sat_mul(ma, oneb + mb);
          if (g.kind == OBX_AGG_SUM_PROD3) {
            if (jc < 0 || !maxabs_of(g.ic, &mc)) return false;
// ... 130 lines not shown
          n_cand++;
          if (axed) n_axed++;
        }
        axes[0] = keep;
        axes[1] = -1;
      }
    }
    if (allow && ok2 && n_cand >= 2 && n_axed >= 1 && axes[0] >= 0) {
      auto axis_dim = [&](int8_t vc) -> uint32_t {
        uint32_t d = st.vdim[vc];
        return d ? d : 1;
      };
      uint32_t d0 = axis_dim(axes[0]);
      uint32_t d1 = axes[1] >= 0 ? axis_dim(axes[1]) : 1;
      const uint32_t cells = st.jcells;
      if ((uint64_t)cells * d0 * d1 * 8 <= 24u * 1024u) {
        st.jws_on = 1;
        st.jws_ja = wja;
        st.jws_a0 = axes[0];
        st.jws_a1 = axes[1];
        st.jws_d0 = d0;
        st.jws_d1 = d1;
        st.jws_cells = cells;
        for (uint32_t a = 0; a < ph.n_aggs; a++) {
          if (!cand[a]) continue;
          st.jws_member[a] = 1;
          const dev_agg &g = ph.aggs[a];
          int8_t tb2[2] = {st.atab_b[a], g.kind == OBX_AGG_SUM_PROD3
                                             ? st.atab_c[a] : (int8_t)-1};
          for (int q = 0; q < 2; q++) {
            if (tb2[q] < 0) continue;
            if ((int8_t)st.tabs[tb2[q]].vc == st.jws_a0)
              st.jws_f0[a] = tb2[q];
            else
              st.jws_f1[a] = tb2[q];
          }
        }
        int nn = 0;
        for (uint32_t a = 0; a < ph.n_aggs; a++) {
          if (st.jws_member[a]) { st.wa64[a] = -1; continue; }
          if (st.wa64[a] >= 0) st.wa64[a] = (int8_t)nn++;
        }
        st.n_w64 = nn;
      }
    }
  }

  {
    const char *ce = getenv("OBX_JIT_CTAB");
    const bool allow = !ce || ce[0] != '0';
    for (uint32_t a = 0; allow && a < ph.n_aggs && st.ctab_agg < 0; a++) {
      const dev_agg &g = ph.aggs[a];
      if (g.kind != OBX_AGG_SUM_PROD3 || st.astrat[a] != JA_I64 ||
          st.jws_member[a] || st.wa64[a] < 0 || st.atab_a[a] >= 0 ||
          st.atab_b[a] < 0 || st.atab_c[a] < 0)
        continue;
      if (a > 0 && (js.agg_f2 & (1u << (a - 1))) && !st.jws_member[a - 1])
        continue;
      const uint16_t ca = ph.need_cols[g.ia], cb = ph.need_cols[g.ib],
                     cc = ph.need_cols[g.ic];
      if (!h.col_known[ca] || !h.col_known[cb] || !h.col_known[cc]) continue;
      const bool empty_b = h.col_min[cb] > h.col_max[cb],
                 empty_c = h.col_min[cc] > h.col_max[cc];
      if (h.col_min[ca] > h.col_max[ca] || empty_b || empty_c) continue;
      if (h.col_min[ca] < 0 || h.col_max[ca] > (int64_t)0xffffffffll)
        continue;
      const __int128 fb_lo = (__int128)g.one_b - h.col_max[cb],
                     fb_hi = (__int128)g.one_b - h.col_min[cb],
                     fc_lo = (__int128)g.one_c + h.col_min[cc],
                     fc_hi = (__int128)g.one_c + h.col_max[cc];
      if (fb_lo < 0 || fc_lo < 0 || fb_hi > 0xffffffffll ||
          fc_hi > 0xffffffffll || fb_hi * fc_hi > 0xffffffffll)
        continue;
      const uint32_t db = st.tabs[st.atab_b[a]].dim,
                     dc = st.tabs[st.atab_c[a]].dim;
      if ((uint64_t)db * dc > 1024) continue;
      st.ctab_agg = (int8_t)a;
      st.ctab_db = db;
      st.ctab_dc = dc;
    }
  }

  if (st.leaf_inline || ph.n_leaves == 0) {
    const char *re = getenv("OBX_JIT_R");
    int r = re ? atoi(re) : 4;
    if (r != 1 && r != 2 && r != 4 && r != 8) r = 4;
    st.r = (uint8_t)r;
    if (st.r > 1) {
      const char *ne = getenv("OBX_JIT_M32");
      const uint32_t w32 = (ne && ne[0] == '0') ? 0 : 32;
      for (uint32_t i = 0; i < ph.n_leaves; i++) {
        const uint32_t rw = h.col_maxw[st.leaf_cols[i]] * st.r;
        st.leaf_multi[i] = rw <= 64 ? 1 : 0;
        st.leaf_m32[i] = rw <= w32 ? 1 : 0;
      }
      for (uint32_t g2 = 0; g2 < ph.n_group_cols; g2++) {
        const uint32_t rw =
            h.col_maxw[ph.need_cols[ph.group_idx[g2]]] * st.r;
        st.g_multi[g2] = rw <= 64 ? 1 : 0;
        st.g_m32[g2] = rw <= w32 ? 1 : 0;
      }
      for (int j = 0; j < js.n_vc; j++) {
        const uint32_t rw = h.col_maxw[js.vcol[j]] * st.r;
        st.v_multi[j] = (st.vmode[j] == JV_REF && rw <= 64) ? 1 : 0;
        st.v_m32[j] = (st.vmode[j] == JV_REF && rw <= w32) ? 1 : 0;
      }
    }
  }
  for (int t = 0; t < st.n_hist; t++)
    if (st.cnt_hist < 0 ||
        st.vdim[st.hist_vc[t]] < st.vdim[st.hist_vc[st.cnt_hist]])
      st.cnt_hist = (int8_t)t;

  if (ph.n_leaves > 0 && !st.leaf_inline) return false;

  {
    const char *se = getenv("OBX_JIT_STRIPES");
    int sn = se ? atoi(se) : 4;
    if (sn != 1 && sn != 2 && sn != 4 && sn != 8 && sn != 16) sn = 4;
    st.stripes = (uint8_t)sn;
  }
  st.stage_bytes = ((h.max_block_len + 24 + 63) / 64) * 64;
  if (st.stage_bytes > OBX_LDS_STAGE_BYTES + 32)
    st.stage_bytes = OBX_LDS_STAGE_BYTES + 32;
  if (st.stage_bytes < st.jcells * ph.n_aggs * 16)
    st.stage_bytes = ((st.jcells * ph.n_aggs * 16 + 63) / 64) * 64;
  uint32_t lds = st.stage_bytes;
  lds += (uint32_t)st.n_w64 * st.jcells * 8 * st.stripes;
  lds += (uint32_t)st.n_mm * st.jcells * 16;
  lds += st.hist_total * 4;
  for (int t = 0; t < st.n_tab; t++) lds += st.tabs[t].dim * 8;
  if (st.ctab_agg >= 0) lds += st.ctab_db * st.ctab_dc * 4;
  lds += 16 * 8 + 16 * 4;
  if (st.jws_on)
    lds += st.jws_cells * st.jws_d0 * st.jws_d1 * 8;
  if (st.cnt_hist < 0) lds += st.jcells * 4 * st.stripes;
  lds += 64;
  st.lds_bytes = lds;
  st.wpb = (int)(163840 / (lds > 1 ? lds : 1));
  if (st.wpb > 8) st.wpb = 8;
  const char *we = getenv("OBX_JIT_WPB");
  if (we) {
    int w = atoi(we);
    if (w >= 2 && w <= 8 && w < st.wpb) st.wpb = w;
  }
  if (st.wpb < 2) return false;
  {
    const uint32_t grid = jit_grid_for(h.n_blocks, h.n_cus, st.wpb);
    const uint64_t maxrows =
        (uint64_t)((h.n_blocks + grid - 1) / grid) *
        (h.max_block_rows ? h.max_block_rows : 4096);
    if (jit_sat_mul(max_term, maxrows) >= BOUND) return false;
  }
  st.ok = true;
  return true;
}

static std::string jit_strategy_sig(const jit_strategy &st) {
  char b[256];
  std::string k = "V2|";
  snprintf(b, sizeof b, "w%dh%dt%dp%dli%dr%dch%ds%du%uc%um%d|",
           st.n_w64, st.n_hist, st.n_tab, st.wpb, st.leaf_inline, st.r,
           st.cnt_hist, st.stripes, st.stage_bytes, st.jcells, st.n_mm);
  k += b;
  for (int i = 0; i < 8; i++) {
    snprintf(b, sizeof b, "m%d%d%d|",
             i < 8 ? st.leaf_multi[i] + 2 * st.leaf_m32[i] : 0,
             i < 2 ? st.g_multi[i] + 2 * st.g_m32[i] : 0,
             i < 4 ? st.v_multi[i] + 2 * st.v_m32[i] : 0);
    k += b;
  }
  for (int i = 0; i < 8; i++) {
    snprintf(b, sizeof b, "L%d:%u|", st.leaf_kind[i], st.leaf_cols[i]);
    k += b;
  }
  for (int j = 0; j < 4; j++) {
    snprintf(b, sizeof b, "v%d:%u:%u:%u|", st.vmode[j], st.vdim[j],
             st.vext[j], st.vraw8[j]);
    k += b;
  }
  for (int a = 0; a < OBX_DEV_MAX_AGGS; a++) {
    snprintf(b, sizeof b, "a%d:%d:%d:%d:%d:%d:%d|", st.astrat[a],
             st.wa64[a], st.ahist[a], st.atab_b[a], st.atab_c[a],
             st.atab_a[a], st.amm[a]);
    k += b;
  }
  for (int t = 0; t < st.n_tab; t++) {
    snprintf(b, sizeof b, "T%u:%u:%lld:%u|", st.tabs[t].vc, st.tabs[t].kind,
             (long long)st.tabs[t].one, st.tabs[t].dim);
    k += b;
  }
  snprintf(b, sizeof b, "C%d:%u:%u|", st.ctab_agg, st.ctab_db, st.ctab_dc);
  k += b;
  if (st.jws_on) {
    snprintf(b, sizeof b, "J%d:%d:%d:%u:%u:%u|", st.jws_ja, st.jws_a0,
             st.jws_a1, st.jws_d0, st.jws_d1, st.jws_cells);
    k += b;
    for (uint32_t a = 0; a < OBX_DEV_MAX_AGGS; a++) {
      snprintf(b, sizeof b, "j%d:%d:%d|", st.jws_member[a], st.jws_f0[a],
               st.jws_f1[a]);
      k += b;
    }
  }
  return k;
}

static std::string jit_gen_source_v2(const dev_plan_hdr &ph,
                                     const jit_shape &js,
                                     const jit_strategy &st) {
  const int NG = ph.n_group_cols;
  const int NL = ph.n_leaves;
  char b[1024];
  std::string s;
  s += "#define OBX_PIPELINE 0\n#include \"obx_dev_common.h\"\n"
       "#include \"obx_jit_dev.h\"\n\n";
  snprintf(b, sizeof b,
           "#define NL %d\n#define NG %d\n#define NW64 %d\n"
           "#define NAGGS %u\n#define HTOT %u\n#define NSTRIPE %u\n"
           "#define JSTAGE %u\n#define JC %u\n\n",
           NL, NG, st.n_w64 > 0 ? st.n_w64 : 1, (unsigned)ph.n_aggs,
           st.hist_total > 0 ? st.hist_total : 1, (unsigned)st.stripes,
           (unsigned)st.stage_bytes, st.jcells);
  s += b;
  snprintf(b, sizeof b,
           "/* Persistent-accumulator scan (the whole-kernel generalization\n"
           "   of the storage group-by pushdown, ObVectorStore::do_group_by):\n"
           "   the dicts are byte-identical in every micro block (verified\n"
           "   at load), so histograms, value tables and group keys are\n"
           "   global-dict-keyed, live in LDS for the kernel's lifetime,\n"
           "   and merge into the global table exactly once. Per block:\n"
           "   stage to LDS, sweep rows, nothing else. */\n"
           "extern \"C\" __global__ __launch_bounds__(256, %d) void "
           "k_jit_scan(\n"
           "    const uint8_t *__restrict__ buf, const dev_block "
           "*__restrict__ blocks,\n"
           "    uint32_t n_blocks, const dev_leaf *__restrict__ "
           "plan_leaves,\n"
           "    const blk_leaf *__restrict__ bleaves, gslot *__restrict__ "
           "gtable,\n"
           "    unsigned long long *__restrict__ counters) {\n",
           st.wpb);
  s += b;
  s += "  __shared__ __attribute__((aligned(16))) uint8_t "
       "lds_blk[JSTAGE];\n";
  s += ""
       "  __shared__ unsigned long long wacc64[NW64][JC][NSTRIPE];\n"
       "  __shared__ uint32_t hist[HTOT];\n";
  if (st.n_mm > 0) {
    snprintf(b, sizeof b,
             "  /* CAS min/max cells: [slot][cell][val, valid] */\n"
             "  __shared__ unsigned long long wmm[%d][JC][2];\n",
             st.n_mm);
    s += b;
  }
  s += ""
       "  __shared__ uint64_t keytab[16];\n"
       "  __shared__ int cslot[16];\n";
  if (st.jws_on) {
    snprintf(b, sizeof b,
             "  __shared__ unsigned long long jws[%uu * %uu * %uu];\n",
             st.jws_cells, st.jws_d0, st.jws_d1);
    s += b;
  }
  if (st.cnt_hist < 0)
    s += "  __shared__ uint32_t wcnt[JC][NSTRIPE];\n";
  for (int t = 0; t < st.n_tab; t++) {
    snprintf(b, sizeof b, "  __shared__ long long vt%d[%u];\n", t,
             st.tabs[t].dim);
    s += b;
  }
  if (st.ctab_agg >= 0) {
    snprintf(b, sizeof b,
             "  /* combined factor table [xb][xc] of the narrowed PROD3 */\n"
             "  __shared__ uint32_t vtc[%uu * %uu];\n",
             st.ctab_db, st.ctab_dc);
    s += b;
  }
  s += "  const uint32_t tid = threadIdx.x, lane = tid & 63, wv = tid >> "
       "6;\n"
       "  uint32_t lane_cnt = 0;\n"
       "  const uint32_t stripe = lane & (NSTRIPE - 1);\n"
       "\n"
       "  for (uint32_t i = tid; i < NW64 * JC * NSTRIPE; i += WG)\n"
       "    (&wacc64[0][0][0])[i] = 0;\n";
  if (st.n_mm > 0) {
    for (uint32_t a = 0; a < ph.n_aggs; a++) {
      if (st.amm[a] < 0) continue;
      snprintf(b, sizeof b,
               "  for (uint32_t i = tid; i < JC; i += WG) {\n"
               "    wmm[%d][i][0] = (unsigned long long)%s;\n"
               "    wmm[%d][i][1] = 0;\n"
               "  }\n",
               st.amm[a],
               ph.aggs[a].kind == OBX_AGG_MIN ? "INT64_MAX" : "INT64_MIN",
               st.amm[a]);
      s += b;
    }
  }
  s += ""
       "  for (uint32_t i = tid; i < HTOT; i += WG) hist[i] = 0;\n";
  if (st.jws_on) {
    snprintf(b, sizeof b,
             "  for (uint32_t i = tid; i < %uu * %uu * %uu; i += WG)\n"
             "    jws[i] = 0;\n",
             st.jws_cells, st.jws_d0, st.jws_d1);
    s += b;
  }
  if (st.cnt_hist < 0)
    s += "  for (uint32_t i = tid; i < JC * NSTRIPE; i += WG)\n"
         "    (&wcnt[0][0])[i] = 0;\n";
  s += "  {\n"
       "    const dev_block &b0 = blocks[0];\n"
       "    blk_view bv0;\n"
       "    bv0.base = buf + b0.block_byte;\n"
       "    bv0.bit_bias = b0.block_byte * 8;\n"
       "    bv0.rbase_bit = 0;\n";
  for (int t = 0; t < st.n_tab; t++) {
    const jit_vtab &vt = st.tabs[t];
    char ex[64];
    if (vt.kind == 0) snprintf(ex, sizeof ex, "e2");
    else if (vt.kind == 1)
      snprintf(ex, sizeof ex, "%lldll - e2", (long long)vt.one);
    else
      snprintf(ex, sizeof ex, "%lldll + e2", (long long)vt.one);
    snprintf(b, sizeof b,
             "    {\n"
             "      const dev_col *tb = &b0.cols[%u];\n"
             "      for (uint32_t e = tid; e <= tb->count && e < %uu; e += "
             "WG) {\n"
             "        long long v2 = 0;\n"
             "        if (e < tb->count) {\n"
             "          long long e2 = dict_entry(bv0, *tb, e);\n"
             "          v2 = %s;\n"
             "        }\n"
             "        vt%d[e] = v2;\n"
             "      }\n"
             "    }\n",
             (unsigned)js.vcol[st.tabs[t].vc], st.tabs[t].dim, ex, t);
    s += b;
  }
  if (st.ctab_agg >= 0) {
    const dev_agg &g = ph.aggs[st.ctab_agg];
    snprintf(b, sizeof b,
             "    {\n"
             "      const dev_col *tb = &b0.cols[%u], *tc = &b0.cols[%u];\n"
             "      for (uint32_t e = tid; e < %uu * %uu; e += WG) {\n"
             "        const uint32_t eb = e / %uu, ec = e %% %uu;\n"
             "        long long fb = 0, fc = 0; /* null slots: factor 0 */\n"
             "        if (eb < tb->count) fb = %lldll - dict_entry(bv0, *tb, "
             "eb);\n"
             "        if (ec < tc->count) fc = %lldll + dict_entry(bv0, *tc, "
             "ec);\n"
             "        vtc[e] = (uint32_t)(fb * fc);\n"
             "      }\n"
             "    }\n",
             (unsigned)ph.need_cols[g.ib], (unsigned)ph.need_cols[g.ic],
             st.ctab_db, st.ctab_dc, st.ctab_dc, st.ctab_dc,
             (long long)g.one_b, (long long)g.one_c);
    s += b;
  }
  if (NG > 0) {
    snprintf(b, sizeof b,
             "    const dev_col *gb0 = &b0.cols[%u];\n"
             "    const uint32_t fdim0 = gb0->count + 1;\n",
             (unsigned)ph.need_cols[ph.group_idx[0]]);
    s += b;
    if (NG > 1) {
      snprintf(b, sizeof b,
               "    const dev_col *gb1 = &b0.cols[%u];\n"
               "    const uint32_t fdim1 = gb1->count + 1;\n"
               "    const uint32_t fcells = fdim0 * fdim1;\n",
               (unsigned)ph.need_cols[ph.group_idx[1]]);
      s += b;
    } else {
      s += "    const uint32_t fcells = fdim0;\n";
    }
    snprintf(b, sizeof b,
             "    for (uint32_t cell = tid; cell < fcells; cell += WG) {\n"
             "      uint32_t r0 = %s;\n"
             "      uint64_t key = 0;\n"
             "      if (r0 >= gb0->count) key |= 1ull << 56;\n"
             "      else {\n"
             "        int64_t kv = dict_entry(bv0, *gb0, r0);\n"
             "        key |= (uint64_t)kv & %s;\n"
             "      }\n",
             NG > 1 ? "cell % fdim0" : "cell",
             ph.group_len[0] >= 8 ? "~0ull"
                                  : "((1ull << (8 * KL0)) - 1)");
    std::string t1(b);
    char kl[16];
    snprintf(kl, sizeof kl, "%u", (unsigned)ph.group_len[0]);
    size_t p;
    while ((p = t1.find("KL0")) != std::string::npos) t1.replace(p, 3, kl);
    s += t1;
    if (NG > 1) {
      snprintf(b, sizeof b,
               "      uint32_t r1 = cell / fdim0;\n"
               "      if (r1 >= gb1->count) key |= 1ull << 57;\n"
               "      else {\n"
               "        int64_t kv1 = dict_entry(bv0, *gb1, r1);\n"
               "        key |= ((uint64_t)kv1 & %s) << (8 * %u);\n"
               "      }\n",
               ph.group_len[1] >= 8 ? "~0ull" : "((1ull << (8 * KL1)) - 1)",
               (unsigned)ph.group_len[0]);
      std::string t2(b);
      snprintf(kl, sizeof kl, "%u", (unsigned)ph.group_len[1]);
      while ((p = t2.find("KL1")) != std::string::npos) t2.replace(p, 3, kl);
      s += t2;
    }
    s += "      keytab[cell] = key;\n"
         "    }\n";
  } else {
    s += "    if (tid == 0) keytab[0] = 0;\n";
  }
  s += "  }\n"
       "  __syncthreads();\n"
       "\n";
  s += "  for (uint32_t blk = blockIdx.x; blk < n_blocks; blk += "
       "gridDim.x) {\n"
       "    const dev_block &cur = blocks[blk];\n"
       "    const blk_leaf *bl = bleaves + (uint64_t)blk * (NL ? NL : "
       "1);\n"
       "    uint8_t blk_verdict = 1;\n"
       "    for (uint32_t i = 0; i < NL; i++) {\n"
       "      uint8_t c = leaf_class(cur, plan_leaves[i], bl[i]);\n"
       "      if (c == 0) { blk_verdict = 0; break; }\n"
       "      if (c == 2) blk_verdict = 2;\n"
       "    }\n"
       "    if (blk_verdict == 0) continue;\n"
       "    __syncthreads(); /* drain previous block's LDS reads */\n"
       "    stage2(buf, cur, lds_blk);\n"
       "    asm volatile(\"s_waitcnt vmcnt(0)\" ::: \"memory\");\n"
       "    __syncthreads();\n";
  s += "    const uint64_t blk_bit = cur.block_byte * 8;\n"
       "    blk_view bv;\n"
       "    bv.base = lds_blk;\n"
       "    bv.bit_bias = blk_bit;\n"
       "    bv.rbase_bit = 0;\n"
       "    const uint32_t rows = cur.row_count;\n"
       "\n";
  if (NG > 0) {
    snprintf(b, sizeof b,
             "    const dev_col *gd0 = &cur.cols[%u];\n"
             "    const uint32_t go0 = (uint32_t)(gd0->data_bit - blk_bit);\n"
             "    const uint32_t gW0 = PW(*gd0);\n"
             "    const uint32_t gn0 = gd0->count;\n",
             (unsigned)ph.need_cols[ph.group_idx[0]]);
    s += b;
  }
  if (NG > 1) {
    snprintf(b, sizeof b,
             "    const dev_col *gd1 = &cur.cols[%u];\n"
             "    const uint32_t go1 = (uint32_t)(gd1->data_bit - blk_bit);\n"
             "    const uint32_t gW1 = PW(*gd1);\n"
             "    const uint32_t gn1 = gd1->count;\n"
             "    const uint32_t dim0 = gn0 + 1;\n",
             (unsigned)ph.need_cols[ph.group_idx[1]]);
    s += b;
  }
  for (int j = 0; j < js.n_vc; j++) {
    if (st.vmode[j] == JV_REF) {
      snprintf(b, sizeof b,
               "    const uint32_t xo%d =\n"
               "        (uint32_t)(cur.cols[%u].data_bit - blk_bit);\n"
               "    const uint32_t xW%d = PW(cur.cols[%u]);\n"
               "    const uint32_t xn%d = cur.cols[%u].count;\n",
               j, (unsigned)js.vcol[j], j, (unsigned)js.vcol[j], j,
               (unsigned)js.vcol[j]);
      s += b;
    } else if (st.vraw8[j]) {
      snprintf(b, sizeof b,
               "    const uint32_t vb%d =\n"
               "        (uint32_t)((cur.cols[%u].data_bit >> 3) - "
               "cur.block_byte);\n",
               j, (unsigned)js.vcol[j]);
      s += b;
    } else {
      snprintf(b, sizeof b,
               "    const col_ctx c%d = make_col_ctx(cur.cols[%u], "
               "blk_bit);\n",
               j, (unsigned)js.vcol[j]);
      s += b;
    }
  }
  for (int i = 0; i < NL; i++) {
    snprintf(b, sizeof b,
             "    const blk_leaf lb%d = bl[%d];\n"
             "    const uint32_t l%do =\n"
             "        (uint32_t)(cur.cols[%u].data_bit - blk_bit);\n"
             "    const uint32_t l%dW = PW(cur.cols[%u]);\n",
             i, i, i, (unsigned)st.leaf_cols[i], i,
             (unsigned)st.leaf_cols[i]);
    s += b;
    if (st.leaf_kind[i] == 1) {
      snprintf(b, sizeof b,
               "    const bool l%d_all = lb%d.mode == OBX_LEAF_ALL;\n", i,
               i);
      s += b;
    }
    if (st.r > 1 && st.leaf_multi[i]) {
      if (st.leaf_m32[i])
        snprintf(b, sizeof b,
                 "    const uint32_t lm%d = (1u << l%dW) - 1;\n", i, i);
      else
        snprintf(b, sizeof b,
                 "    const uint64_t lm%d = (1ull << l%dW) - 1;\n", i, i);
      s += b;
    }
  }
  if (st.r > 1) {
    if (NG > 0 && st.g_multi[0])
      s += st.g_m32[0] ? "    const uint32_t gm0 = (1u << gW0) - 1;\n"
                          : "    const uint64_t gm0 = (1ull << gW0) - 1;\n";
    if (NG > 1 && st.g_multi[1])
      s += st.g_m32[1] ? "    const uint32_t gm1 = (1u << gW1) - 1;\n"
                          : "    const uint64_t gm1 = (1ull << gW1) - 1;\n";
    for (int j = 0; j < js.n_vc; j++)
      if (st.v_multi[j]) {
        if (st.v_m32[j])
          snprintf(b, sizeof b,
                   "    const uint32_t xm%d = (1u << xW%d) - 1;\n", j, j);
        else
          snprintf(b, sizeof b,
                   "    const uint64_t xm%d = (1ull << xW%d) - 1;\n", j, j);
        s += b;
      }
  }

  std::string acc;
  acc += "        lane_cnt += live ? 1u : 0u;\n";
  acc += "        if (live) {\n";
  if (st.cnt_hist < 0)
    acc += "          atomicAdd(&wcnt[cell][stripe], 1u);\n";
  for (int t = 0; t < st.n_hist; t++) {
    int j = st.hist_vc[t];
    snprintf(b, sizeof b,
             "          atomicAdd(&hist[%uu + cell * %uu + x%d], 1u);\n",
             st.hist_off[t], st.vdim[j], j);
    acc += b;
  }
  if (st.jws_on) {
    char idx[224];
    if (st.jws_a1 >= 0)
      snprintf(idx, sizeof idx,
               "cell * %uu + (x%d < %uu ? x%d : %uu) * %uu + (x%d < %uu ? "
               "x%d : %uu)",
               st.jws_d0 * st.jws_d1, st.jws_a0, st.jws_d0, st.jws_a0,
               st.jws_d0 - 1, st.jws_d1, st.jws_a1, st.jws_d1, st.jws_a1,
               st.jws_d1 - 1);
    else
      snprintf(idx, sizeof idx, "cell * %uu + (x%d < %uu ? x%d : %uu)",
               st.jws_d0, st.jws_a0, st.jws_d0, st.jws_a0, st.jws_d0 - 1);
    snprintf(b, sizeof b,
             "          if (!nu%d)\n"
             "            atomicAdd(&jws[%s],\n"
             "                      (unsigned long long)v%d);\n",
             st.jws_ja, idx, st.jws_ja);
    acc += b;
  }
  for (uint32_t a = 0; a < ph.n_aggs; a++) {
    const dev_agg &g = ph.aggs[a];
    if (st.jws_member[a]) continue;
    if (st.astrat[a] == JA_I64_COUNT) {
      snprintf(b, sizeof b,
               "          if (!nu%d)\n"
               "            atomicAdd(&wacc64[%d][cell][stripe], 1ull);\n",
               st.aval_a[a], st.wa64[a]);
      acc += b;
      continue;
    }
    if (st.astrat[a] == JA_MM) {
      snprintf(b, sizeof b,
               "          if (!nu%d) {\n"
               "            cas_minmax(&wmm[%d][cell][0], v%d, %s);\n"
               "            wmm[%d][cell][1] = 1;\n"
               "          }\n",
               st.aval_a[a], st.amm[a], st.aval_a[a],
               g.kind == OBX_AGG_MIN ? "true" : "false", st.amm[a]);
      acc += b;
      continue;
    }
    if (st.astrat[a] != JA_I64) continue;
    int ja = st.aval_a[a];
    char va[64];
    if (st.atab_a[a] >= 0)
      snprintf(va, sizeof va, "vt%d[x%d]", st.atab_a[a], ja);
    else
      snprintf(va, sizeof va, "v%d", ja);
    auto slot_lookup = [&](uint8_t need_idx) -> int {
      for (int j2 = 0; j2 < js.n_vc; j2++)
        if (js.vcol[j2] == ph.need_cols[need_idx]) return j2;
      return -1;
    };
    switch (g.kind) {
      case OBX_AGG_SUM:
        snprintf(b, sizeof b,
                 "          atomicAdd(&wacc64[%d][cell][stripe],\n"
                 "                    (unsigned long long)%s);\n",
                 st.wa64[a], va);
        acc += b;
        break;
      case OBX_AGG_SUM_MUL: {
        int jb = slot_lookup(g.ib);
        char vb[64];
        if (st.atab_b[a] >= 0)
          snprintf(vb, sizeof vb, "vt%d[x%d]", st.atab_b[a], jb);
        else
          snprintf(vb, sizeof vb, "(nu%d ? 0ll : v%d)", jb, jb);
        snprintf(b, sizeof b,
                 "          atomicAdd(&wacc64[%d][cell][stripe],\n"
                 "                    (unsigned long long)((long long)%s * "
                 "%s));\n",
                 st.wa64[a], va, vb);
        acc += b;
        break;
      }
      case OBX_AGG_SUM_PROD2: {
        int jb = slot_lookup(g.ib);
        char vb[64];
        if (st.atab_b[a] >= 0)
          snprintf(vb, sizeof vb, "vt%d[x%d]", st.atab_b[a], jb);
        else
          snprintf(vb, sizeof vb, "(nu%d ? 0ll : (%lldll - v%d))", jb,
                   (long long)g.one_b, jb);
        snprintf(b, sizeof b,
                 "          long long p2_%u = (long long)%s * %s;\n"
                 "          atomicAdd(&wacc64[%d][cell][stripe],\n"
                 "                    (unsigned long long)p2_%u);\n",
                 a, va, vb, st.wa64[a], a);
        acc += b;
        if ((js.agg_f2 & (1u << a)) && !st.jws_member[a + 1]) {
          const dev_agg &g3 = ph.aggs[a + 1];
          int jc = slot_lookup(g3.ic);
          char vc[64];
          if (st.atab_c[a + 1] >= 0)
            snprintf(vc, sizeof vc, "vt%d[x%d]", st.atab_c[a + 1], jc);
          else
            snprintf(vc, sizeof vc, "(nu%d ? 0ll : (%lldll + v%d))", jc,
                     (long long)g3.one_c, jc);
          snprintf(b, sizeof b,
                   "          atomicAdd(&wacc64[%d][cell][stripe],\n"
                   "                    (unsigned long long)(p2_%u * "
                   "%s));\n",
                   st.wa64[a + 1], a, vc);
          acc += b;
// ... 483 lines not shown
```

oceanbase_amd/csrc/obx_kernels.hip:

```cpp
#include "obx_dev_common.h"

struct prog_spec { uint8_t n; uint8_t t[15]; };

__device__ __forceinline__ void filter_prog_phase(
    const blk_view bv, const dev_block &cur,
    const dev_leaf *__restrict__ plan_leaves,
    const blk_leaf *__restrict__ bl, uint32_t n_leaves, prog_spec ps,
    uint32_t rows, uint32_t w0, uint64_t blk_bit, lds3_u64 *pass_bm,
    lds3_u64 *leaf_bm_flat) {
  const uint32_t tid = threadIdx.x;
  const uint32_t lane = tid & 63;
  const uint32_t wv = tid >> 6;
  const uint32_t iters = (rows + WG - 1) / WG;
  uint8_t cls[8];
  for (uint32_t i = 0; i < n_leaves; i++) {
    cls[i] = leaf_class(cur, plan_leaves[i], bl[i]);
    if (cls[i] != 2) continue;
    leaf_ctx lc = make_leaf_ctx(cur, plan_leaves[i], bl[i], blk_bit);
    const bool slow = lc.slow;
    for (uint32_t it = 0; it < iters; it++) {
      uint32_t rr = it * WG + tid;
      uint32_t r = w0 + rr;
      bool pass = rr < rows;
      if (pass)
// ... 819 lines not shown
      if (lo > hi) { out.mode = OBX_LEAF_NONE; return; }
      out.mode = OBX_LEAF_RANGE; out.lo = (uint64_t)lo; out.hi = (uint64_t)hi;
      return;
    }
    default:
      out.mode = OBX_LEAF_VALUE;
      return;
  }
}

extern "C" __global__ void k_lower_leaves(
    const uint8_t *__restrict__ buf, const dev_block *__restrict__ blocks,
    uint32_t n_blocks, const dev_leaf *__restrict__ pl, uint32_t n_leaves,
    uint32_t n_cols, const int64_t *__restrict__ minmax,
    blk_leaf *__restrict__ out) {
  uint64_t idx = (uint64_t)blockIdx.x * blockDim.x + threadIdx.x;
  uint64_t total = (uint64_t)n_blocks * n_leaves;
  if (idx >= total) return;
  uint32_t b = (uint32_t)(idx / n_leaves);
  uint32_t i = (uint32_t)(idx % n_leaves);
  const dev_leaf &lf = pl[i];
  const dev_col &c = blocks[b].cols[lf.col];
  blk_view bv; bv.base = buf; bv.bit_bias = 0; bv.rbase_bit = 0;
  blk_leaf o;
  o.mask = 0; o.lo = 0; o.hi = 0; o.mode = OBX_LEAF_VALUE; o.invert = 0;

  if (lf.op == 10) {
    const dev_col &bc = blocks[b].cols[lf.bcols[0]];
    if (lf.n_bcols == 1 &&
        (bc.enc == OBX_D_DICT || bc.enc == OBX_D_RLE) && bc.count < 64) {
      for (uint32_t e = 0; e < bc.count; e++) {
        int64_t v = dict_entry(bv, bc, e);
        bool nu0 = false;
        if (black_eval_vals(lf, &v, &nu0)) o.mask |= 1ull << e;
      }
      o.mode = (o.mask == 0) ? OBX_LEAF_NONE : OBX_LEAF_REF_MASK;
    } else if (lf.n_bcols == 1 && bc.enc == OBX_D_CONST && bc.runs == 0) {
      int64_t v = bc.base;
      bool nu0 = (bc.count == 0);
      o.mode = black_eval_vals(lf, &v, &nu0) ? OBX_LEAF_ALL : OBX_LEAF_NONE;
    } else {
      o.mode = OBX_LEAF_VALUE;
    }
    out[idx] = o;
    return;
  }

  const bool is_dict = (c.enc == OBX_D_DICT || c.enc == OBX_D_RLE);
  if (is_dict && c.count < 64) {
    if (lf.op == 8) {
      o.mask = 1ull << c.count;
    } else if (lf.op == 9) {
      o.mask = (c.count == 0) ? 0 : ((1ull << c.count) - 1);
    } else {
      for (uint32_t e = 0; e < c.count; e++) {
        int64_t v = dict_entry(bv, c, e);
        if (leaf_value_match(lf, v, false)) o.mask |= 1ull << e;
      }
    }
    o.mode = (o.mask == 0) ? OBX_LEAF_NONE : OBX_LEAF_REF_MASK;
  } else if (c.enc == OBX_D_RAW && (c.flags & OBX_DF_BITPACK) && lf.op <= 6) {
    uint64_t dmax = (c.width >= 64) ? ~0ull : ((1ull << c.width) - 1);
    lower_range((__int128)lf.vlo, (__int128)lf.vhi, lf.op, dmax, o);
  } else if (c.enc == OBX_D_RAW && !(c.flags & OBX_DF_BITPACK) &&
             !(c.flags & OBX_DF_STRING) && lf.op <= 6 && lf.op != 7 ) {
    uint32_t kbits = (uint32_t)c.width * 8;
    uint64_t dmax = (kbits >= 64) ? ~0ull : ((1ull << kbits) - 1);
    bool signed_dom = ((c.flags & OBX_DF_SIGNED) && c.width >= c.tss) ||
                      (!(c.flags & OBX_DF_SIGNED) && c.width == 8);
    if (signed_dom) {
      uint64_t bias = 1ull << (kbits - 1);
      __int128 smin = -(__int128)bias, smax = (__int128)bias - 1;
      auto biasmap = [&](int64_t x) -> __int128 {
        __int128 v = x;
        if (v < smin) return (__int128)-1;
        if (v > smax) return (__int128)dmax + 1;
        return v + (__int128)bias;
      };
      lower_range(biasmap(lf.vlo), biasmap(lf.vhi), lf.op, dmax, o);
      if (o.mode == OBX_LEAF_RANGE) o.mask = bias;
    } else {
      lower_range((__int128)lf.vlo, (__int128)lf.vhi, lf.op, dmax, o);
    }
  } else if (c.enc == OBX_D_INTDIFF && lf.op <= 6) {
    uint32_t kbits = (c.flags & OBX_DF_BITPACK) ? c.width : c.width * 8;
    uint64_t dmax = (kbits >= 64) ? ~0ull : ((1ull << kbits) - 1);
    lower_range((__int128)lf.vlo - c.base, (__int128)lf.vhi - c.base, lf.op,
                dmax, o);
  } else if ((c.enc == OBX_D_RAW || c.enc == OBX_D_INTDIFF) &&
             (lf.op == 8 || lf.op == 9)) {
    if (c.flags & OBX_DF_HAS_EXT) {
      o.mode = OBX_LEAF_NULL;
      o.invert = (lf.op == 9);
    } else {
      o.mode = (lf.op == 8) ? OBX_LEAF_NONE : OBX_LEAF_ALL;
    }
  } else if (c.enc == OBX_D_CONST && c.runs == 0) {
    bool isn = (c.count == 0);
    bool m = leaf_value_match(lf, c.base, isn);
    o.mode = m ? OBX_LEAF_ALL : OBX_LEAF_NONE;
  } else {
    o.mode = OBX_LEAF_VALUE;
  }

  if (minmax && lf.op <= 6 && !(c.flags & OBX_DF_STRING) &&
      (o.mode == OBX_LEAF_RANGE || o.mode == OBX_LEAF_VALUE)) {
    int64_t mn = minmax[2 * ((uint64_t)b * n_cols + lf.col)];
    int64_t mx = minmax[2 * ((uint64_t)b * n_cols + lf.col) + 1];
    if (!(mn == INT64_MIN && mx == INT64_MAX)) {
      bool none = false, all = false;
      if (mn > mx) {
        none = true;
      } else {
        const int64_t lo = lf.vlo, hi = lf.vhi;
        switch (lf.op) {
          case 0: none = lo < mn || lo > mx; all = (mn == mx && mn == lo);
                  break;
          case 1: none = mn > lo; all = mx <= lo; break;
          case 2: none = mn >= lo; all = mx < lo; break;
          case 3: none = mx < lo; all = mn >= lo; break;
          case 4: none = mx <= lo; all = mn > lo; break;
          case 5: none = (mn == mx && mn == lo); all = lo < mn || lo > mx;
                  break;
          case 6: none = mx < lo || mn > hi; all = mn >= lo && mx <= hi;
                  break;
        }
      }
      if (none) o.mode = OBX_LEAF_NONE;
      else if (all) o.mode = OBX_LEAF_ALL;
    }
  }
  out[idx] = o;
}

extern "C" __global__ void k_gtable_init(
    unsigned long long *__restrict__ words, uint32_t n_slots,
    uint32_t tail_words, uint32_t min_mask, uint32_t max_mask) {
  const uint32_t SW = (uint32_t)(sizeof(gslot) / 8);
  const uint32_t total = n_slots * SW + tail_words;
  const uint32_t i = blockIdx.x * blockDim.x + threadIdx.x;
  if (i >= total) return;
  unsigned long long v = 0;
  if (i < n_slots * SW) {
    const uint32_t w = i % SW;
    if (w == 0) {
      v = OBX_KEY_EMPTY;
    } else if (w >= 2 && ((w - 2) & 3) == 0) {
      const uint32_t a = (w - 2) >> 2;
      if ((min_mask >> a) & 1) v = (unsigned long long)INT64_MAX;
      else if ((max_mask >> a) & 1) v = (unsigned long long)INT64_MIN;
    }
  }
  words[i] = v;
}

extern "C" __global__ void k_col_minmax(
    const uint8_t *__restrict__ buf, const dev_block *__restrict__ blocks,
    uint32_t n_blocks, uint32_t n_cols, int64_t *__restrict__ out) {
  const uint32_t lane = threadIdx.x & 63;
  const uint32_t wv = threadIdx.x >> 6;
  uint64_t total = (uint64_t)n_blocks * n_cols;
  for (uint64_t wid = (uint64_t)blockIdx.x * WAVES + wv; wid < total;
       wid += (uint64_t)gridDim.x * WAVES) {
    uint32_t b = (uint32_t)(wid / n_cols), c = (uint32_t)(wid % n_cols);
    const dev_block &blk = blocks[b];
    const dev_col &dc = blk.cols[c];
    blk_view bv;
    bv.base = buf;
    bv.bit_bias = 0;
    bv.rbase_bit = 0;
    int64_t mn = INT64_MAX, mx = INT64_MIN;
    bool known = true;
    if (dc.flags & OBX_DF_STRING) {
      known = false;
    } else {
      switch (dc.enc) {
        case OBX_D_DICT:
        case OBX_D_RLE:
          for (uint32_t e = lane; e < dc.count; e += 64) {
            int64_t v = dict_entry(bv, dc, e);
            if (v < mn) mn = v;
            if (v > mx) mx = v;
          }
          break;
        case OBX_D_CONST:
          if (dc.runs == 0) {
            if (lane == 0 && dc.count) mn = mx = dc.base;
          } else {
            for (uint32_t e = lane; e < dc.count; e += 64) {
              int64_t v = dict_entry(bv, dc, e);
              if (v < mn) mn = v;
              if (v > mx) mx = v;
            }
          }
          break;
        case OBX_D_RAW:
        case OBX_D_INTDIFF:
          for (uint32_t r = lane; r < blk.row_count; r += 64) {
            bool isn;
            int64_t v = col_value(bv, dc, r, isn);
            if (!isn) {
              if (v < mn) mn = v;
              if (v > mx) mx = v;
            }
          }
          break;
        default:
          known = false;
          break;
      }
    }
    if (!known) {
      mn = INT64_MIN;
      mx = INT64_MAX;
    }
    for (int off = 32; off > 0; off >>= 1) {
      int64_t omn = (int64_t)shflxor64((uint64_t)mn, off);
      int64_t omx = (int64_t)shflxor64((uint64_t)mx, off);
      if (known) {
        if (omn < mn) mn = omn;
        if (omx > mx) mx = omx;
      }
    }
    if (lane == 0) {
      out[2 * wid] = mn;
      out[2 * wid + 1] = mx;
    }
  }
}


__device__ __forceinline__ int g_slot(gslot *gtable, uint64_t key) {
  uint32_t idx = (uint32_t)((key * 0x9E3779B97F4A7C15ull) >> (64 - OBX_GTABLE_SHIFT)) &
                 (OBX_GTABLE_SLOTS - 1);
  for (int probe = 0; probe < OBX_GTABLE_SLOTS; probe++) {
    unsigned long long k = __hip_atomic_load(
        &gtable[idx].key, __ATOMIC_RELAXED, __HIP_MEMORY_SCOPE_AGENT);
    if (k == key) return (int)idx;
    if (k == OBX_KEY_EMPTY) {
      unsigned long long cur = atomicCAS(&gtable[idx].key, OBX_KEY_EMPTY,
                                         (unsigned long long)key);
      if (cur == OBX_KEY_EMPTY || cur == key) return (int)idx;
    }
    idx = (idx + 1) & (OBX_GTABLE_SLOTS - 1);
  }
  return -1;
}

__device__ __forceinline__ bool pass_bit(const uint64_t *__restrict__ bitmap,
                                         uint64_t grow) {
  return (bitmap[grow >> 6] >> (grow & 63)) & 1;
}

extern "C" __global__ __launch_bounds__(WG, 2) void k_group_pass(
    const uint8_t *__restrict__ buf, const dev_block *__restrict__ blocks,
    uint32_t n_blocks, const dev_plan_hdr ph,
    const uint64_t *__restrict__ bitmap, uint8_t *__restrict__ row_slot,
    gslot *__restrict__ gtable, unsigned long long *__restrict__ counters) {
  __shared__ uint8_t cell_slot[64];
  __shared__ unsigned long long cnt[OBX_GTABLE_SLOTS][4];
  const uint32_t tid = threadIdx.x;
  const uint32_t lane = tid & 63;

  for (uint32_t i = tid; i < OBX_GTABLE_SLOTS; i += WG) {
    cnt[i][0] = 0; cnt[i][1] = 0; cnt[i][2] = 0; cnt[i][3] = 0;
  }
  __syncthreads();

  for (uint32_t b = blockIdx.x; b < n_blocks; b += gridDim.x) {
    const dev_block &cur = blocks[b];
    const uint64_t blk_bit = cur.block_byte * 8;
    blk_view bv;
    bv.base = buf; bv.bit_bias = 0; bv.rbase_bit = blk_bit;
    const uint32_t rows = cur.row_count;
    const uint64_t row_start = dev_block_row_start(&cur);

    col_ctx g0, g1;
    const dev_col *gd0 = nullptr, *gd1 = nullptr;
    if (ph.n_group_cols > 0) {
      gd0 = &cur.cols[ph.need_cols[ph.group_idx[0]]];
      g0 = make_col_ctx(*gd0, blk_bit);
    }
    if (ph.n_group_cols > 1) {
      gd1 = &cur.cols[ph.need_cols[ph.group_idx[1]]];
      g1 = make_col_ctx(*gd1, blk_bit);
    }
    const uint32_t kl0 = ph.group_len[0], kl1 = ph.group_len[1];
    const uint32_t dim0 = (ph.n_group_cols > 0) ? g0.count + 1 : 1;
    const uint32_t dim1 = (ph.n_group_cols > 1) ? g1.count + 1 : 1;
    const bool ref_fast = ph.n_group_cols > 0 && g0.kind == 1 &&
                          (ph.n_group_cols < 2 || g1.kind == 1) &&
                          dim0 * dim1 <= 64;
    if (ref_fast) {
      __syncthreads();
      for (uint32_t i = tid; i < 64; i += WG) cell_slot[i] = 254;
      __syncthreads();
    }

    const uint32_t iters = (rows + WG - 1) / WG;
    for (uint32_t it = 0; it < iters; it++) {
      uint32_t r = it * WG + tid;
      bool in = r < rows;
      bool pass = in && pass_bit(bitmap, row_start + r);
      uint8_t slot8 = 255;
      if (pass) {
        if (ref_fast) {
// ... 291 lines not shown
```

oceanbase_amd/engine.py:

```python
import ctypes as C
import os

from . import abi

_PKG = os.path.dirname(os.path.abspath(__file__))
_SO = os.path.join(_PKG, "libobx.so")

OBX_NO_GPU = -7001


class EngineUnavailable(RuntimeError):
    pass


def _load():
    if not os.path.exists(_SO):
        raise EngineUnavailable(
            f"{_SO} not built — run oceanbase_amd/csrc/build.sh (the product "
            "path has no CPU fallback)")
    lib = C.CDLL(_SO)
    lib.obx_gpu_open.restype = C.c_int
    lib.obx_gpu_open.argtypes = [C.c_int, C.POINTER(C.c_void_p)]
    lib.obx_gpu_close.restype = C.c_int
    lib.obx_gpu_close.argtypes = [C.c_void_p]
    lib.obx_gpu_load_blocks.restype = C.c_int
    lib.obx_gpu_load_blocks.argtypes = [C.c_void_p, C.POINTER(abi.BlockSet)]
    lib.obx_gpu_load_cs_blocks.restype = C.c_int
    lib.obx_gpu_load_cs_blocks.argtypes = [C.c_void_p,
                                           C.POINTER(abi.BlockSet)]
    lib.obx_gpu_free_blocks.restype = C.c_int
    lib.obx_gpu_free_blocks.argtypes = [C.c_void_p, C.c_int]
    lib.obx_gpu_filter.restype = C.c_int
    lib.obx_gpu_filter.argtypes = [C.c_void_p, C.c_int,
                                   C.POINTER(abi.FilterDesc), C.c_int]
    lib.obx_gpu_fetch_bitmap.restype = C.c_int
    lib.obx_gpu_fetch_bitmap.argtypes = [C.c_void_p, C.c_int, C.c_void_p,
                                         C.c_int64]
    lib.obx_gpu_fetch_row_ids.restype = C.c_int
    lib.obx_gpu_fetch_row_ids.argtypes = [C.c_void_p, C.c_int, C.c_void_p,
                                          C.c_int64, C.POINTER(C.c_uint64)]
    lib.obx_gpu_fetch_blk_counts.restype = C.c_int
    lib.obx_gpu_fetch_blk_counts.argtypes = [C.c_void_p, C.c_int, C.c_void_p,
                                             C.c_int64]
    lib.obx_gpu_decode.restype = C.c_int
    lib.obx_gpu_decode.argtypes = [C.c_void_p, C.c_int,
                                   C.POINTER(C.c_uint16), C.c_uint16]
    lib.obx_gpu_fetch_col.restype = C.c_int
    lib.obx_gpu_fetch_col.argtypes = [C.c_void_p, C.c_int, C.c_uint16,
                                      C.c_void_p, C.c_int64]
    lib.obx_gpu_scan_project.restype = C.c_int
    lib.obx_gpu_scan_project.argtypes = [C.c_void_p, C.c_int,
                                         C.POINTER(abi.FilterDesc),
                                         C.POINTER(C.c_uint16), C.c_uint16,
                                         C.c_int, C.POINTER(C.c_uint64)]
    lib.obx_gpu_fetch_proj.restype = C.c_int
    lib.obx_gpu_fetch_proj.argtypes = [C.c_void_p, C.c_int, C.c_uint16,
                                       C.c_uint64, C.c_uint64, C.c_void_p,
                                       C.c_int64, C.c_void_p, C.c_int64,
                                       C.POINTER(C.c_uint64)]
    lib.obx_gpu_fetch_proj_row_nos.restype = C.c_int
    lib.obx_gpu_fetch_proj_row_nos.argtypes = [C.c_void_p, C.c_int,
                                               C.c_uint64, C.c_uint64,
                                               C.c_void_p, C.c_int64,
                                               C.POINTER(C.c_uint64)]
    lib.obx_gpu_last_proj_stage_ms.restype = C.c_double
    lib.obx_gpu_last_proj_stage_ms.argtypes = [C.c_void_p, C.c_int]
    lib.obx_gpu_scan_filter_agg.restype = C.c_int
    lib.obx_gpu_scan_filter_agg.argtypes = [C.c_void_p, C.c_int,
                                            C.POINTER(abi.FilterDesc),
                                            C.POINTER(abi.AggDesc),
                                            C.POINTER(abi.AggResult)]
    lib.obx_gpu_last_kernel_ms.restype = C.c_double
    lib.obx_gpu_last_kernel_ms.argtypes = [C.c_void_p]
    lib.obx_gpu_last_prep_ms.restype = C.c_double
    lib.obx_gpu_last_prep_ms.argtypes = [C.c_void_p]
    lib.obx_gpu_last_jit.restype = C.c_int
    lib.obx_gpu_last_jit.argtypes = [C.c_void_p]
    for f in ("obx_gpu_total_rows", "obx_gpu_total_bytes",
              "obx_gpu_last_survivors"):
        getattr(lib, f).restype = C.c_uint64
        getattr(lib, f).argtypes = [C.c_void_p, C.c_int]
    return lib


_lib = None


def lib():
    global _lib
    if _lib is None:
        _lib = _load()
    return _lib


class GpuEngine:
    def __init__(self, device=0):
        self._lib = lib()
        self._ctx = C.c_void_p()
        rc = self._lib.obx_gpu_open(device, C.byref(self._ctx))
        if rc == OBX_NO_GPU:
            raise EngineUnavailable("no HIP device visible (product path "
                                    "refuses to run without a GPU)")
        if rc != 0:
            raise RuntimeError(f"obx_gpu_open failed: {rc}")

    def close(self):
        if self._ctx:
            self._lib.obx_gpu_close(self._ctx)
            self._ctx = None

    def __del__(self):
        try:
            self.close()
        except Exception:
            pass

    def load(self, bs):
        h = self._lib.obx_gpu_load_blocks(self._ctx, C.byref(bs))
        if h < 0:
            raise RuntimeError(f"obx_gpu_load_blocks failed: {h}")
        return h

    def load_cs(self, cs_blocks, schema):
        from . import cs as _cs
        bs, keep = _cs.make_blockset(cs_blocks, schema)
        h = self._lib.obx_gpu_load_cs_blocks(self._ctx, C.byref(bs))
        if h < 0:
            raise RuntimeError(f"obx_gpu_load_cs_blocks failed: {h}")
        return h

    def free(self, handle):
        self._lib.obx_gpu_free_blocks(self._ctx, handle)

    def filter(self, handle, filter_desc, want_row_ids=False):
        rc = self._lib.obx_gpu_filter(self._ctx, handle,
                                      C.byref(filter_desc),
                                      1 if want_row_ids else 0)
        if rc != 0:
            raise RuntimeError(f"obx_gpu_filter failed: {rc}")
        return self._lib.obx_gpu_last_survivors(self._ctx, handle)

    def fetch_bitmap(self, handle):
        import numpy as np
        rows = self._lib.obx_gpu_total_rows(self._ctx, handle)
        out = np.zeros((rows + 7) // 8, dtype=np.uint8)
        rc = self._lib.obx_gpu_fetch_bitmap(self._ctx, handle,
                                            out.ctypes.data_as(C.c_void_p),
                                            out.nbytes)
        if rc != 0:
            raise RuntimeError(f"fetch_bitmap failed: {rc}")
        return out

    def fetch_row_ids(self, handle):
        import numpy as np
        rows = self._lib.obx_gpu_total_rows(self._ctx, handle)
        out = np.zeros(rows, dtype=np.int32)
        n = C.c_uint64(0)
        rc = self._lib.obx_gpu_fetch_row_ids(self._ctx, handle,
                                             out.ctypes.data_as(C.c_void_p),
                                             rows, C.byref(n))
        if rc != 0:
            raise RuntimeError(f"fetch_row_ids failed: {rc}")
        return out, int(n.value)

    def fetch_blk_counts(self, handle, n_blocks):
        import numpy as np
        out = np.zeros(n_blocks, dtype=np.uint32)
        rc = self._lib.obx_gpu_fetch_blk_counts(
            self._ctx, handle, out.ctypes.data_as(C.c_void_p), n_blocks)
        if rc != 0:
            raise RuntimeError(f"fetch_blk_counts failed: {rc}")
        return out

    def decode(self, handle, cols):
        arr = (C.c_uint16 * len(cols))(*cols)
        rc = self._lib.obx_gpu_decode(self._ctx, handle, arr, len(cols))
        if rc != 0:
            raise RuntimeError(f"obx_gpu_decode failed: {rc}")

    def fetch_col(self, handle, col, datum_len):
        import numpy as np
        rows = self._lib.obx_gpu_total_rows(self._ctx, handle)
        out = np.zeros(rows * datum_len, dtype=np.uint8)
        rc = self._lib.obx_gpu_fetch_col(self._ctx, handle, col,
                                         out.ctypes.data_as(C.c_void_p),
                                         out.nbytes)
        if rc != 0:
            raise RuntimeError(f"fetch_col failed: {rc}")
        return out

    def scan_project(self, handle, filter_desc, cols, want_row_nos=False):
        arr = (C.c_uint16 * len(cols))(*cols)
        n = C.c_uint64(0)
        rc = self._lib.obx_gpu_scan_project(
            self._ctx, handle,
            C.byref(filter_desc) if filter_desc is not None else None,
            arr, len(cols), 1 if want_row_nos else 0, C.byref(n))
        if rc != 0:
            raise RuntimeError(f"obx_gpu_scan_project failed: {rc}")
        return int(n.value)

    def _proj_window(self, handle, proj_idx, start, count):
        n = C.c_uint64(0)
        rc = self._lib.obx_gpu_fetch_proj(
            self._ctx, handle, proj_idx, start,
            count if count is not None else 2**63, None, 0, None, 0,
            C.byref(n))
        if rc != 0:
            raise RuntimeError(f"obx_gpu_fetch_proj failed: {rc}")
        return int(n.value)

    def fetch_proj(self, handle, proj_idx, datum_len, start=0, count=None):
        import numpy as np
        n = self._proj_window(handle, proj_idx, start, count)
        out = np.zeros(n * datum_len, dtype=np.uint8)
        nulls = np.zeros((n + 7) // 8, dtype=np.uint8)
        got = C.c_uint64(0)
        rc = self._lib.obx_gpu_fetch_proj(
            self._ctx, handle, proj_idx, start, n,
            out.ctypes.data_as(C.c_void_p), out.nbytes,
            nulls.ctypes.data_as(C.c_void_p), nulls.nbytes, C.byref(got))
        if rc != 0:
            raise RuntimeError(f"obx_gpu_fetch_proj failed: {rc}")
        assert got.value == n
        return out, nulls

    def fetch_proj_row_nos(self, handle, start=0, count=None):
        import numpy as np
        n = C.c_uint64(0)
        rc = self._lib.obx_gpu_fetch_proj_row_nos(
# ... 71 lines not shown
```

Baseline: 234.6 billion rows/s.

## Pack per-block column metadata into compact cached descriptors for JIT scan

Adds a 128-byte per-block descriptor that packs the block offset, length, row count and the needed columns' bit offset, count, width and flags into single u64 slots. A small kernel builds it, and it is cached per column set on the handle. The JIT v2 scan kernel loads this compact descriptor plus the block's leaf words up front and skips pruned blocks before staging, instead of reading the wide dev_block struct. This is meant to cut metadata load traffic and latency in the block loop. The cost is an extra build kernel on first use (counted as prep time), extra device memory, and an optional OBX_JIT_SGRID grid cap knob.

```diff
diff --git a/include/obx.h b/include/obx.h
--- a/include/obx.h
+++ b/include/obx.h
@@ -235,6 +235,8 @@
 double obx_gpu_last_kernel_ms(obx_gpu_ctx *ctx);
 double obx_gpu_last_prep_ms(obx_gpu_ctx *ctx);
 int obx_gpu_last_jit(obx_gpu_ctx *ctx);
+int obx_gpu_last_bdesc(obx_gpu_ctx *ctx);
+int64_t obx_gpu_bdesc_builds(obx_gpu_ctx *ctx, int handle);
 uint32_t obx_gpu_last_grid(obx_gpu_ctx *ctx);
 uint64_t obx_gpu_total_rows(obx_gpu_ctx *ctx, int handle);
 uint64_t obx_gpu_total_bytes(obx_gpu_ctx *ctx, int handle);
diff --git a/oceanbase_amd/csrc/obx_dev.h b/oceanbase_amd/csrc/obx_dev.h
--- a/oceanbase_amd/csrc/obx_dev.h
+++ b/oceanbase_amd/csrc/obx_dev.h
@@ -126,6 +126,57 @@
 
 #define OBX_DEV_MAX_NEED 12
 
+typedef struct __attribute__((aligned(128))) obx_bdesc {
+  uint64_t block_byte;
+  uint32_t block_len;
+  uint32_t row_count;
+  uint64_t slot[OBX_DEV_MAX_NEED];
+  uint64_t pad[2];
+} obx_bdesc;
+
+typedef struct obx_bdesc_cols {
+  uint16_t c[OBX_DEV_MAX_NEED];
+  uint32_t n;
+} obx_bdesc_cols;
+
+#define OBX_BD_OFF(s) ((uint32_t)(s))
+#define OBX_BD_COUNT(s) ((uint32_t)((s) >> 32) & 0xFFFFu)
+#define OBX_BD_WIDTH(s) ((uint32_t)((s) >> 48) & 0xFFu)
+#define OBX_BD_FLAGS(s) ((uint32_t)((s) >> 56))
+
+#if defined(__HIPCC__) || defined(__HIP_DEVICE_COMPILE__)
+__host__ __device__
+#endif
+static inline int obx_bdesc_pack_col(const dev_col *c, uint64_t block_byte,
+                                     uint64_t *slot) {
+  const uint32_t w = (c->flags & OBX_DF_BITPACK) ? (uint32_t)c->width
+                                                 : (uint32_t)c->width * 8u;
+  const uint32_t off = (uint32_t)(c->data_bit - block_byte * 8);
+  const int fits = c->count <= 0xFFFFu && w <= 0xFFu;
+  *slot = (uint64_t)off | ((uint64_t)(c->count & 0xFFFFu) << 32) |
+          ((uint64_t)(w & 0xFFu) << 48) | ((uint64_t)c->flags << 56);
+  return fits;
+}
+
+#if defined(__HIPCC__) || defined(__HIP_DEVICE_COMPILE__)
+__host__ __device__
+#endif
+static inline int obx_bdesc_pack(const dev_block *b, const uint16_t *cols,
+                                 uint32_t n_cols, obx_bdesc *out) {
+  int fits = 1;
+  out->block_byte = b->block_byte;
+  out->block_len = b->block_len;
+  out->row_count = b->row_count;
+  for (uint32_t i = 0; i < OBX_DEV_MAX_NEED; i++) {
+    out->slot[i] = 0;
+    if (i < n_cols)
+      fits &= obx_bdesc_pack_col(&b->cols[cols[i]], b->block_byte,
+                                 &out->slot[i]);
+  }
+  out->pad[0] = out->pad[1] = 0;
+  return fits;
+}
+
 typedef struct dev_pass_agg {
   uint8_t kind;
   uint8_t agg_idx;
diff --git a/oceanbase_amd/csrc/obx_engine.cpp b/oceanbase_amd/csrc/obx_engine.cpp
--- a/oceanbase_amd/csrc/obx_engine.cpp
+++ b/oceanbase_amd/csrc/obx_engine.cpp
@@ -19,6 +19,8 @@
   HIP_TRY(hipEventCreate(&ctx->ev_p0));
   HIP_TRY(hipEventCreate(&ctx->ev_p1));
   HIP_TRY(hipEventCreate(&ctx->ev_mid));
+  HIP_TRY(hipEventCreate(&ctx->ev_b0));
+  HIP_TRY(hipEventCreate(&ctx->ev_b1));
   {
     hipDeviceProp_t prop;
     HIP_TRY(hipGetDeviceProperties(&prop, device));
@@ -37,7 +39,7 @@
   ctx->handles.clear();
   (void)hipStreamDestroy(ctx->stream);
   for (hipEvent_t ev : {ctx->ev_start, ctx->ev_stop, ctx->ev_p0, ctx->ev_p1,
-                        ctx->ev_mid})
+                        ctx->ev_mid, ctx->ev_b0, ctx->ev_b1})
     (void)hipEventDestroy(ev);
   (void)hipHostFree(ctx->h_result);
   delete ctx;
@@ -55,6 +57,8 @@
     if (p) (void)hipFree(p);
   for (uint8_t *p : d_sel_out)
     if (p) (void)hipFree(p);
+  for (bdesc_set &s : bdesc)
+    if (s.d) (void)hipFree(s.d);
 }
 
 static obx_handle *lookup(obx_gpu_ctx *ctx, int handle) {
@@ -79,6 +83,10 @@
 static uint32_t jit_grid_for(uint32_t n_blocks, uint32_t n_cus, int wpb) {
   uint64_t g = (uint64_t)(n_cus ? n_cus : 1) * (uint32_t)(wpb > 0 ? wpb : 1) *
                OBX_JIT_GRID_WAVES;
+  if (const char *sg = getenv("OBX_JIT_SGRID")) {
+    const long v = atol(sg);
+    if (v >= 1 && (uint64_t)v < g) g = (uint64_t)v;
+  }
   if (g > n_blocks) g = n_blocks;
   return g ? (uint32_t)g : 1;
 }
@@ -152,6 +160,9 @@
     if (dc.enc == OBX_D_RAW || dc.enc == OBX_D_DICT || dc.enc == OBX_D_INTDIFF)
       w = (dc.flags & OBX_DF_BITPACK) ? dc.width : (uint32_t)dc.width * 8;
     if (w > h.col_maxw[c]) h.col_maxw[c] = w;
+    uint64_t slot;
+    if (!obx_bdesc_pack_col(&dc, db.block_byte, &slot))
+      h.col_bdesc_unfit[c] = true;
   }
   summarize_col_classes(h);
   if (db.row_count > h.max_block_rows) h.max_block_rows = db.row_count;
@@ -710,6 +721,37 @@
   return OBX_SUCCESS;
 }
 
+static const obx_bdesc *bdesc_get(obx_handle &h, const obx_bdesc_cols &cols,
+                                  hipStream_t stream, bool *built) {
+  *built = false;
+  obx_handle::bdesc_set *victim = nullptr;
+  for (obx_handle::bdesc_set &s : h.bdesc) {
+    if (s.d && s.cols.n == cols.n &&
+        memcmp(s.cols.c, cols.c, cols.n * sizeof(cols.c[0])) == 0)
+      return s.d;
+    if (!victim || (victim->d && (!s.d || s.born < victim->born)))
+      victim = &s;
+  }
+  if (victim->d) {
+    (void)hipFree(victim->d);
+    victim->d = nullptr;
+  }
+  const uint64_t nb = h.n_blocks ? h.n_blocks : 1;
+  if (hipMalloc(&victim->d, nb * sizeof(obx_bdesc)) != hipSuccess) {
+    victim->d = nullptr;
+    return nullptr;
+  }
+  victim->cols = cols;
+  victim->born = ++h.bdesc_builds;
+  const uint64_t words = (uint64_t)h.n_blocks * 16;
+  hipLaunchKernelGGL(k_pack_bdesc,
+                     dim3((uint32_t)((words + OBX_WG_HOST - 1) / OBX_WG_HOST)),
+                     dim3(OBX_WG_HOST), 0, stream, h.d_blocks, h.n_blocks,
+                     cols, victim->d);
+  *built = true;
+  return victim->d;
+}
+
 #include "obx_jit.inc"
 
 static decltype(&k_filter) generic_filter_kernel(const obx_handle &h,
@@ -731,6 +773,11 @@
   if (prep) {
     HIP_TRY(hipEventElapsedTime(&ms, ctx->ev_p0, ctx->ev_p1));
     ctx->last_prep_ms = ms;
+    if (ctx->bdesc_built) {
+      ctx->bdesc_built = false;
+      HIP_TRY(hipEventElapsedTime(&ms, ctx->ev_b0, ctx->ev_b1));
+      ctx->last_prep_ms += ms;
+    }
   }
   return OBX_SUCCESS;
 }
@@ -1086,6 +1133,8 @@
   if (rc != OBX_SUCCESS) return rc;
   ctx->last_jit = 0;
   ctx->last_grid = 0;
+  ctx->last_bdesc = 0;
+  ctx->bdesc_built = false;
 
   uint32_t min_mask = 0, max_mask = 0;
   for (uint32_t a = 0; a < ph.n_aggs; a++) {
@@ -1127,9 +1176,17 @@
   } else {
     jit_entry *je = jit_prepare(h, ph, plv);
     ctx->last_jit = je ? g_jit_kind : 0;
+    const obx_bdesc *bd = nullptr;
+    if (je && je->bdesc) {
+      HIP_TRY(hipEventRecord(ctx->ev_b0, ctx->stream));
+      bd = bdesc_get(h, je->bd_cols, ctx->stream, &ctx->bdesc_built);
+      if (!bd) return OBX_INTERNAL_ERROR;
+      HIP_TRY(hipEventRecord(ctx->ev_b1, ctx->stream));
+    }
+    ctx->last_bdesc = bd != nullptr;
     HIP_TRY(hipEventRecord(ctx->ev_start, ctx->stream));
     if (je) {
-      if (jit_launch(je, h, ctx->stream, &ctx->last_grid) != 0)
+      if (jit_launch(je, h, bd, ctx->stream, &ctx->last_grid) != 0)
         return OBX_INTERNAL_ERROR;
     } else {
       auto kfn = h.lds_ok
@@ -1254,6 +1311,7 @@
     h.col_max[c] = col_max[c];
     h.col_maxcnt[c] = col_maxcnt[c];
     h.col_maxw[c] = col_maxw ? col_maxw[c] : 255;
+    h.col_bdesc_unfit[c] = col_maxcnt[c] > 0xFFFFu;
     uint8_t cls = h.col_dict_every[c] ? 1 : 0;
     if (obx_store_class(cols[c].obj_type) == OBX_SC_STRING) cls |= 0x10;
     h.col_class.push_back(cls);
@@ -1345,13 +1403,14 @@
                           h.lds_ok, h.max_block_rows, h.max_block_len};
   memcpy(handle_out, hf, sizeof(hf));
   for (uint16_t c = 0; c < h.n_cols; c++) {
-    const bool f[9] = {h.col_dict_every[c], h.col_dict_any[c],
-                       h.col_dict_stable[c], h.col_grp16_every[c],
-                       h.col_raw8_every[c], h.col_rangefam_every[c],
-                       h.col_ext_any[c], h.col_slow_any[c], h.col_span_any[c]};
+    const bool f[10] = {h.col_dict_every[c], h.col_dict_any[c],
+                        h.col_dict_stable[c], h.col_grp16_every[c],
+                        h.col_raw8_every[c], h.col_rangefam_every[c],
+                        h.col_ext_any[c], h.col_slow_any[c], h.col_span_any[c],
+                        h.col_bdesc_unfit[c]};
     uint32_t *o = col_out + 4 * c;
     o[0] = 0;
-    for (int i = 0; i < 9; i++) o[0] |= (uint32_t)f[i] << i;
+    for (int i = 0; i < 10; i++) o[0] |= (uint32_t)f[i] << i;
     o[1] = h.col_maxcnt[c];
     o[2] = h.col_maxw[c];
     o[3] = h.col_cnt_max[c];
@@ -1369,6 +1428,24 @@
 
 extern "C" int obx_gpu_last_jit(obx_gpu_ctx *ctx) {
   return ctx ? ctx->last_jit : 0;
+}
+
+extern "C" int obx_gpu_last_bdesc(obx_gpu_ctx *ctx) {
+  return ctx ? ctx->last_bdesc : 0;
+}
+
+extern "C" int64_t obx_gpu_bdesc_builds(obx_gpu_ctx *ctx, int handle) {
+  obx_handle *h = lookup(ctx, handle);
+  return h ? (int64_t)h->bdesc_builds : -1;
+}
+
+extern "C" int obx_bdesc_probe(const dev_block *blk, const uint16_t *cols,
+                               uint32_t n_cols, obx_bdesc *out) {
+  if (!blk || !cols || !out || n_cols > OBX_DEV_MAX_NEED)
+    return OBX_INVALID_ARGUMENT;
+  for (uint32_t i = 0; i < n_cols; i++)
+    if (cols[i] >= OBX_DEV_MAX_COLS) return OBX_INVALID_ARGUMENT;
+  return obx_bdesc_pack(blk, cols, n_cols, out);
 }
 
 extern "C" uint32_t obx_gpu_last_grid(obx_gpu_ctx *ctx) {
diff --git a/oceanbase_amd/csrc/obx_host.h b/oceanbase_amd/csrc/obx_host.h
--- a/oceanbase_amd/csrc/obx_host.h
+++ b/oceanbase_amd/csrc/obx_host.h
@@ -3,6 +3,7 @@
 
 #include <hip/hip_runtime.h>
 
+#include <cstddef>
 #include <cstdio>
 #include <map>
 #include <memory>
@@ -69,6 +70,11 @@
     const uint8_t *, const dev_block *, uint32_t, uint32_t, int64_t *);
 extern "C" __global__ void k_gtable_init(
     unsigned long long *, uint32_t, uint32_t, uint32_t, uint32_t);
+extern "C" __global__ void k_pack_bdesc(const dev_block *, uint32_t,
+                                        const obx_bdesc_cols, obx_bdesc *);
+static_assert(sizeof(obx_bdesc) == 128 && alignof(obx_bdesc) == 128 &&
+                  offsetof(obx_bdesc, slot) == 16,
+              "k_pack_bdesc writes obx_bdesc as 16 u64 words");
 
 extern "C" __global__ void k_project_tile_sums(const uint32_t *, uint32_t,
                                                uint64_t *);
@@ -163,6 +169,15 @@
   bool col_rangefam_every[OBX_DEV_MAX_COLS] = {};
   uint32_t col_maxcnt[OBX_DEV_MAX_COLS] = {};
   uint32_t col_maxw[OBX_DEV_MAX_COLS] = {};
+  bool col_bdesc_unfit[OBX_DEV_MAX_COLS] = {};
+
+#define OBX_BDESC_SETS 4
+  struct bdesc_set {
+    obx_bdesc_cols cols = {};
+    obx_bdesc *d = nullptr;
+    uint64_t born = 0;
+  } bdesc[OBX_BDESC_SETS];
+  uint64_t bdesc_builds = 0;
 
   int64_t *d_minmax = nullptr;
   int64_t col_min[OBX_DEV_MAX_COLS] = {};
@@ -176,9 +191,12 @@
   hipEvent_t ev_start = nullptr, ev_stop = nullptr;
   hipEvent_t ev_p0 = nullptr, ev_p1 = nullptr;
   hipEvent_t ev_mid = nullptr;
+  hipEvent_t ev_b0 = nullptr, ev_b1 = nullptr;
+  bool bdesc_built = false;
   double last_ms = 0.0;
   double last_prep_ms = 0.0;
   int last_jit = 0;
+  int last_bdesc = 0;
   double last_proj_ms[3] = {0.0, 0.0, 0.0};
   uint32_t last_grid = 0;
   uint32_t n_cus = 256;
diff --git a/oceanbase_amd/csrc/obx_jit.inc b/oceanbase_amd/csrc/obx_jit.inc
--- a/oceanbase_amd/csrc/obx_jit.inc
+++ b/oceanbase_amd/csrc/obx_jit.inc
@@ -8,6 +8,8 @@
   hipModule_t mod = nullptr;
   hipFunction_t fn = nullptr;
   int wpb = 0;
+  bool bdesc = false;
+  obx_bdesc_cols bd_cols = {};
 };
 
 struct jit_shape {
@@ -173,12 +175,17 @@
   jit_build_strategy(h, ph, js, pl, st);
   if (!st.ok && js.has_mm) return nullptr;
   g_jit_kind = st.ok ? 2 : 1;
-  return jit_get(
+  jit_entry *je = jit_get(
       jit_plan_sig(ph) + (st.ok ? jit_strategy_sig(st) : "V1|"),
       [&] {
         return st.ok ? jit_gen_source_v2(ph, js, st) : jit_gen_source(ph, js);
       },
       "k_jit_scan", "obx_jit_src.hip", st.ok ? st.wpb : 0);
+  if (je && st.ok) {
+    je->bdesc = st.bdesc != 0;
+    je->bd_cols = st.bd_cols;
+  }
+  return je;
 }
 
 static jit_entry *jit_prepare_filter(const obx_handle &h,
@@ -199,13 +206,13 @@
       "k_jit_filter", "obx_jit_filter_src.hip", 0);
 }
 
-static int jit_launch(jit_entry *je, obx_handle &h, hipStream_t stream,
-                      uint32_t *grid_out) {
+static int jit_launch(jit_entry *je, obx_handle &h, const obx_bdesc *bd,
+                      hipStream_t stream, uint32_t *grid_out) {
   const uint32_t grid = je->wpb ? jit_grid_for(h.n_blocks, h.n_cus, je->wpb)
                                 : grid_for(h.n_blocks);
   *grid_out = grid;
-  void *args[7] = {&h.d_buf,     &h.d_blocks, &h.n_blocks, &h.d_pleaves,
-                   &h.d_bleaves, &h.d_gtable, &h.d_counters};
+  void *args[8] = {&h.d_buf,     &h.d_blocks, &h.n_blocks,   &h.d_pleaves,
+                   &h.d_bleaves, &h.d_gtable, &h.d_counters, &bd};
   return hipModuleLaunchKernel(je->fn, grid, 1, 1, OBX_WG_HOST, 1, 1, 0,
                                stream, args, nullptr) == hipSuccess
              ? 0
diff --git a/oceanbase_amd/csrc/obx_jit_dev.h b/oceanbase_amd/csrc/obx_jit_dev.h
--- a/oceanbase_amd/csrc/obx_jit_dev.h
+++ b/oceanbase_amd/csrc/obx_jit_dev.h
@@ -6,10 +6,10 @@
                                  : (uint32_t)(dc).width * 8u)
 
 __device__ __forceinline__ void stage2(
-    const uint8_t *__restrict__ buf, const dev_block &blk,
+    const uint8_t *__restrict__ buf, uint64_t block_byte, uint32_t block_len,
     uint8_t *dst) {
-  const uint32_t n16 = (blk.block_len + 15) >> 4;
-  const uint8_t *src = buf + blk.block_byte;
+  const uint32_t n16 = (block_len + 15) >> 4;
+  const uint8_t *src = buf + block_byte;
   for (uint32_t i = threadIdx.x; i < n16; i += WG) {
     __builtin_amdgcn_global_load_lds(
         (const __attribute__((address_space(1))) uint32_t
@@ -18,6 +18,43 @@
              *)(dst + (size_t)i * 16),
         16, 0, 0);
   }
+}
+
+__device__ __forceinline__ void stage2(
+    const uint8_t *__restrict__ buf, const dev_block &blk,
+    uint8_t *dst) {
+  stage2(buf, blk.block_byte, blk.block_len, dst);
+}
+
+struct jit_leafw {
+  uint64_t mask, lo, hi, mi;
+};
+typedef uint64_t __attribute__((may_alias)) jit_u64a;
+__device__ __forceinline__ jit_leafw jit_load_leafw(
+    const blk_leaf *__restrict__ p) {
+  const jit_u64a *w = (const jit_u64a *)p;
+  jit_leafw l;
+  l.mask = w[0];
+  l.lo = w[1];
+  l.hi = w[2];
+  l.mi = w[3];
+  return l;
+}
+__device__ __forceinline__ blk_leaf jit_leaf_of(const jit_leafw &w) {
+  blk_leaf l;
+  l.mask = w.mask;
+  l.lo = w.lo;
+  l.hi = w.hi;
+  l.mode = (uint8_t)w.mi;
+  l.invert = (uint8_t)(w.mi >> 8);
+  return l;
+}
+__device__ __forceinline__ uint8_t jit_leaf_class(const jit_leafw &w,
+                                                  uint32_t col_flags) {
+  const uint8_t mode = (uint8_t)w.mi;
+  if (mode == OBX_LEAF_NONE) return 0;
+  if (mode == OBX_LEAF_ALL && !(col_flags & OBX_DF_HAS_EXT)) return 1;
+  return 2;
 }
 
 __device__ __forceinline__ uint64_t jit_bread(
diff --git a/oceanbase_amd/csrc/obx_jit_scan.inc b/oceanbase_amd/csrc/obx_jit_scan.inc
--- a/oceanbase_amd/csrc/obx_jit_scan.inc
+++ b/oceanbase_amd/csrc/obx_jit_scan.inc
@@ -66,7 +66,15 @@
   uint32_t ctab_db = 0, ctab_dc = 0;
   uint32_t lds_bytes = 0;
   int wpb = 7;
+  uint8_t bdesc = 0;
+  obx_bdesc_cols bd_cols = {};
 };
+
+static int jit_bd_slot(const jit_strategy &st, uint16_t col) {
+  for (uint32_t i = 0; i < st.bd_cols.n; i++)
+    if (st.bd_cols.c[i] == col) return (int)i;
+  return -1;
+}
 
 static bool jit_col_maxabs(const obx_handle &h, uint16_t col, uint64_t *out) {
   if (!h.col_known[col]) return false;
@@ -503,6 +511,26 @@
         (h.max_block_rows ? h.max_block_rows : 4096);
     if (jit_sat_mul(max_term, maxrows) >= BOUND) return false;
   }
+  {
+    const char *be = getenv("OBX_JIT_BDESC");
+    bool on = !be || be[0] != '0';
+    obx_bdesc_cols bc = {};
+    auto add = [&](uint16_t col) {
+      for (uint32_t i = 0; i < bc.n; i++)
+        if (bc.c[i] == col) return;
+      if (bc.n >= OBX_DEV_MAX_NEED || h.col_bdesc_unfit[col]) {
+        on = false;
+        return;
+      }
+      bc.c[bc.n++] = col;
+    };
+    for (uint32_t i = 0; on && i < ph.n_need; i++) add(ph.need_cols[i]);
+    for (uint32_t i = 0; on && i < ph.n_leaves; i++) add(st.leaf_cols[i]);
+    if (on) {
+      st.bdesc = 1;
+      st.bd_cols = bc;
+    }
+  }
   st.ok = true;
   return true;
 }
@@ -543,6 +571,13 @@
   }
   snprintf(b, sizeof b, "C%d:%u:%u|", st.ctab_agg, st.ctab_db, st.ctab_dc);
   k += b;
+  snprintf(b, sizeof b, "B%d", st.bdesc);
+  k += b;
+  for (uint32_t i = 0; i < st.bd_cols.n; i++) {
+    snprintf(b, sizeof b, ":%u", st.bd_cols.c[i]);
+    k += b;
+  }
+  k += "|";
   if (st.jws_on) {
     snprintf(b, sizeof b, "J%d:%d:%d:%u:%u:%u|", st.jws_ja, st.jws_a0,
              st.jws_a1, st.jws_d0, st.jws_d1, st.jws_cells);
@@ -556,12 +591,76 @@
   return k;
 }
 
+static void jit_gen_block_head_bdesc(const dev_plan_hdr &ph,
+                                     const jit_shape &js,
+                                     const jit_strategy &st, std::string &s) {
+  const int NG = ph.n_group_cols;
+  const int NL = ph.n_leaves;
+  char b[1024];
+  s += "  for (uint32_t blk = blockIdx.x; blk < n_blocks; blk += "
+       "gridDim.x) {\n"
+       "    jmeta cm;\n"
+       "    jit_load_meta(cm, bdesc, bleaves, blk);\n"
+       "    uint8_t blk_verdict = 1;\n";
+  for (int i = 0; i < NL; i++) {
+    snprintf(b, sizeof b,
+             "    {\n"
+             "      const uint8_t c = jit_leaf_class(\n"
+             "          cm.lf[%d], OBX_BD_FLAGS(cm.s[%d]));\n"
+             "      if (c == 0) blk_verdict = 0;\n"
+             "      else if (c == 2 && blk_verdict) blk_verdict = 2;\n"
+             "    }\n",
+             i, jit_bd_slot(st, st.leaf_cols[i]));
+    s += b;
+  }
+  s += "    if (blk_verdict == 0) continue;\n"
+       "    __syncthreads(); /* drain previous block's LDS reads */\n"
+       "    stage2(buf, cm.byte, cm.len, lds_blk);\n"
+       "    asm volatile(\"s_waitcnt vmcnt(0)\" ::: \"memory\");\n"
+       "    __syncthreads();\n"
+       "    const uint64_t blk_bit = cm.byte * 8;\n"
+       "    blk_view bv;\n"
+       "    bv.base = lds_blk;\n"
+       "    bv.bit_bias = blk_bit;\n"
+       "    bv.rbase_bit = 0;\n"
+       "    const uint32_t rows = cm.rows;\n"
+       "\n";
+  for (int g = 0; g < NG && g < 2; g++) {
+    const int k = jit_bd_slot(st, ph.need_cols[ph.group_idx[g]]);
+    snprintf(b, sizeof b,
+             "    const uint32_t go%d = OBX_BD_OFF(cm.s[%d]);\n"
+             "    const uint32_t gW%d = OBX_BD_WIDTH(cm.s[%d]);\n"
+             "    const uint32_t gn%d = OBX_BD_COUNT(cm.s[%d]);\n",
+             g, k, g, k, g, k);
+    s += b;
+  }
+  if (NG > 1) s += "    const uint32_t dim0 = gn0 + 1;\n";
+  for (int j = 0; j < js.n_vc; j++) {
+    const int k = jit_bd_slot(st, js.vcol[j]);
+    if (st.vmode[j] == JV_REF)
+      snprintf(b, sizeof b,
+               "    const uint32_t xo%d = OBX_BD_OFF(cm.s[%d]);\n"
+               "    const uint32_t xW%d = OBX_BD_WIDTH(cm.s[%d]);\n"
+               "    const uint32_t xn%d = OBX_BD_COUNT(cm.s[%d]);\n",
+               j, k, j, k, j, k);
+    else if (st.vraw8[j])
+      snprintf(b, sizeof b,
+               "    const uint32_t vb%d = OBX_BD_OFF(cm.s[%d]) >> 3;\n", j, k);
+    else
+      snprintf(b, sizeof b,
+               "    const col_ctx c%d =\n"
+               "        make_col_ctx(blocks[blk].cols[%u], blk_bit);\n",
+               j, (unsigned)js.vcol[j]);
+    s += b;
+  }
+}
+
 static std::string jit_gen_source_v2(const dev_plan_hdr &ph,
                                      const jit_shape &js,
                                      const jit_strategy &st) {
   const int NG = ph.n_group_cols;
   const int NL = ph.n_leaves;
-  char b[1024];
+  char b[2048];
   std::string s;
   s += "#define OBX_PIPELINE 0\n#include \"obx_dev_common.h\"\n"
        "#include \"obx_jit_dev.h\"\n\n";
@@ -573,6 +672,36 @@
            st.hist_total > 0 ? st.hist_total : 1, (unsigned)st.stripes,
            (unsigned)st.stage_bytes, st.jcells);
   s += b;
+  if (st.bdesc) {
+    snprintf(b, sizeof b,
+             "#define NBS %u\n"
+             "/* what the block loop needs of one block, in registers: the\n"
+             "   packed descriptor's header and column slots, and the\n"
+             "   block's lowered leaf tests. Wave-uniform, whole words:\n"
+             "   scalar loads. */\n"
+             "struct jmeta {\n"
+             "  uint64_t byte;\n"
+             "  uint32_t len, rows;\n"
+             "  uint64_t s[NBS];\n"
+             "  jit_leafw lf[NL ? NL : 1];\n"
+             "};\n"
+             "__device__ __forceinline__ void jit_load_meta(\n"
+             "    jmeta &m, const obx_bdesc *__restrict__ bdesc,\n"
+             "    const blk_leaf *__restrict__ bleaves, uint32_t blk) {\n"
+             "  const obx_bdesc &d = bdesc[blk];\n"
+             "  m.byte = d.block_byte;\n"
+             "  m.len = d.block_len;\n"
+             "  m.rows = d.row_count;\n"
+             "#pragma unroll\n"
+             "  for (uint32_t i = 0; i < NBS; i++) m.s[i] = d.slot[i];\n"
+             "#pragma unroll\n"
+             "  for (uint32_t i = 0; i < NL; i++)\n"
+             "    m.lf[i] = jit_load_leafw(bleaves + (uint64_t)blk * NL + "
+             "i);\n"
+             "}\n\n",
+             st.bd_cols.n);
+    s += b;
+  }
   snprintf(b, sizeof b,
            "/* Persistent-accumulator scan (the whole-kernel generalization\n"
            "   of the storage group-by pushdown, ObVectorStore::do_group_by):\n"
@@ -589,7 +718,8 @@
            "plan_leaves,\n"
            "    const blk_leaf *__restrict__ bleaves, gslot *__restrict__ "
            "gtable,\n"
-           "    unsigned long long *__restrict__ counters) {\n",
+           "    unsigned long long *__restrict__ counters,\n"
+           "    const obx_bdesc *__restrict__ bdesc) {\n",
            st.wpb);
   s += b;
   s += "  __shared__ __attribute__((aligned(16))) uint8_t "
@@ -767,6 +897,9 @@
   s += "  }\n"
        "  __syncthreads();\n"
        "\n";
+  if (st.bdesc) {
+    jit_gen_block_head_bdesc(ph, js, st, s);
+  } else {
   s += "  for (uint32_t blk = blockIdx.x; blk < n_blocks; blk += "
        "gridDim.x) {\n"
        "    const dev_block &cur = blocks[blk];\n"
@@ -834,14 +967,24 @@
       s += b;
     }
   }
+  }
   for (int i = 0; i < NL; i++) {
-    snprintf(b, sizeof b,
-             "    const blk_leaf lb%d = bl[%d];\n"
-             "    const uint32_t l%do =\n"
-             "        (uint32_t)(cur.cols[%u].data_bit - blk_bit);\n"
-             "    const uint32_t l%dW = PW(cur.cols[%u]);\n",
-             i, i, i, (unsigned)st.leaf_cols[i], i,
-             (unsigned)st.leaf_cols[i]);
+    if (st.bdesc) {
+      const int k = jit_bd_slot(st, st.leaf_cols[i]);
+      snprintf(b, sizeof b,
+               "    const blk_leaf lb%d = jit_leaf_of(cm.lf[%d]);\n"
+               "    const uint32_t l%do = OBX_BD_OFF(cm.s[%d]);\n"
+               "    const uint32_t l%dW = OBX_BD_WIDTH(cm.s[%d]);\n",
+               i, i, i, k, i, k);
+    } else {
+      snprintf(b, sizeof b,
+               "    const blk_leaf lb%d = bl[%d];\n"
+               "    const uint32_t l%do =\n"
+               "        (uint32_t)(cur.cols[%u].data_bit - blk_bit);\n"
+               "    const uint32_t l%dW = PW(cur.cols[%u]);\n",
+               i, i, i, (unsigned)st.leaf_cols[i], i,
+               (unsigned)st.leaf_cols[i]);
+    }
     s += b;
     if (st.leaf_kind[i] == 1) {
       snprintf(b, sizeof b,
diff --git a/oceanbase_amd/csrc/obx_kernels.hip b/oceanbase_amd/csrc/obx_kernels.hip
--- a/oceanbase_amd/csrc/obx_kernels.hip
+++ b/oceanbase_amd/csrc/obx_kernels.hip
@@ -995,6 +995,21 @@
     }
   }
   words[i] = v;
+}
+
+extern "C" __global__ void k_pack_bdesc(
+    const dev_block *__restrict__ blocks, uint32_t n_blocks,
+    const obx_bdesc_cols cols, obx_bdesc *__restrict__ out) {
+  const uint64_t i = (uint64_t)blockIdx.x * blockDim.x + threadIdx.x;
+  const uint32_t blk = (uint32_t)(i >> 4), w = (uint32_t)i & 15;
+  if (blk >= n_blocks) return;
+  const dev_block &b = blocks[blk];
+  uint64_t v = 0;
+  if (w == 0) v = b.block_byte;
+  else if (w == 1) v = (uint64_t)b.block_len | ((uint64_t)b.row_count << 32);
+  else if (w - 2 < cols.n)
+    (void)obx_bdesc_pack_col(&b.cols[cols.c[w - 2]], b.block_byte, &v);
+  ((uint64_t *)out)[i] = v;
 }
 
 extern "C" __global__ void k_col_minmax(
diff --git a/oceanbase_amd/engine.py b/oceanbase_amd/engine.py
--- a/oceanbase_amd/engine.py
+++ b/oceanbase_amd/engine.py
@@ -76,6 +76,10 @@
     lib.obx_gpu_last_prep_ms.argtypes = [C.c_void_p]
     lib.obx_gpu_last_jit.restype = C.c_int
     lib.obx_gpu_last_jit.argtypes = [C.c_void_p]
+    lib.obx_gpu_last_bdesc.restype = C.c_int
+    lib.obx_gpu_last_bdesc.argtypes = [C.c_void_p]
+    lib.obx_gpu_bdesc_builds.restype = C.c_int64
+    lib.obx_gpu_bdesc_builds.argtypes = [C.c_void_p, C.c_int]
     for f in ("obx_gpu_total_rows", "obx_gpu_total_bytes",
               "obx_gpu_last_survivors"):
         getattr(lib, f).restype = C.c_uint64
```

Result: faster. 248.0 billion rows/s (median of 6 runs) (+5.7%).
